# kcroker/Gadget-2.0.7-ngravs

Measured on AMD Instinct MI355X. Metric: particle-steps/s (tree+PM), higher is better.
Workload: dtype f64

## Files before the change

gadget-2.0.7-ngravs_amd/__init__.py:

```python
import ctypes as C
import os
import subprocess

import numpy as np

from . import abi, ic
from .abi import (Config, Particles, Stats, make_config, WALK_GROUP, WALK_STRICT,
                  LAW_NONE, LAW_NEWTON, LAW_NEG_NEWTON, LAW_YUKAWA, LAW_COLOYUK, LAW_BAMBAM, LAW_SOURCEBAM, LAW_TARGETBAM)

_HERE = os.path.dirname(os.path.abspath(__file__))
LIB_PATH = os.path.join(_HERE, "libngravs_hip.so")
_LIB = None

EXPORTS = [
    "ngravs_abi_version", "ngravs_build_info", "ngravs_config_default", "ngravs_create", "ngravs_create_with_laws", "ngravs_destroy",
    "ngravs_last_walk_kernel", "ngravs_last_pm_cus", "ngravs_cu_probe", "ngravs_shortrange_table_with_laws", "ngravs_user_table_eval",
    "ngravs_create_with_lattice", "ngravs_user_lattice_table",
    "ngravs_set_fatal_handler", "ngravs_set_opening", "ngravs_set_walk_mode", "ngravs_set_softening", "ngravs_dd_record_bytes", "ngravs_get_config", "ngravs_set_tuning",
    "ngravs_memcpy", "ngravs_device_alloc", "ngravs_device_free",
    "ngravs_set_particles",
    "ngravs_set_old_acc", "ngravs_update_particles", "ngravs_force_update_tree", "ngravs_domain_decomposition", "ngravs_discard_grav_pm",
    "ngravs_force_treebuild", "ngravs_gravity_tree",
    "ngravs_pmforce_periodic", "ngravs_compute_accelerations", "ngravs_get_accel", "ngravs_get_stats", "ngravs_walk_unopened",
    "ngravs_get_domain", "ngravs_get_keys", "ngravs_get_order", "ngravs_get_shard", "ngravs_last_error",
    "ngravs_peano_hilbert_key", "ngravs_peano_keys", "ngravs_shortrange_table", "ngravs_direct_sum", "ngravs_direct_sum_targets",
    "ngravs_dd_num_local", "ngravs_dd_local_extent", "ngravs_dd_set_extent", "ngravs_get_domain_extent", "ngravs_dd_set_toptree",
    "ngravs_dd_get_toptree", "ngravs_dd_peano_order", "ngravs_dd_leaf_sums", "ngravs_dd_target_bounds", "ngravs_dd_keep_margin", "ngravs_dd_pack", "ngravs_dd_get_dest",
    "ngravs_dd_pack_leaves", "ngravs_dd_set_top", "ngravs_dd_recv_buffer", "ngravs_dd_apply_migration", "ngravs_dd_set_halo",
    "ngravs_dd_leaf_sums_kept", "ngravs_dd_pack_leaves_kept", "ngravs_dd_refresh_halo", "ngravs_dd_update_top", "ngravs_dd_get_kept",
    "ngravs_dd_set_ids", "ngravs_dd_get_ids",
    "ngravs_pm_slab_begin", "ngravs_pm_slab_pack", "ngravs_pm_slab_unpack", "ngravs_pm_slab_bytes",
    "ngravs_sph_density", "ngravs_sph_kernel", "ngravs_sph_hydro",
]
HOST_EXPORTS = ["ngravs_host_comm_selftest", "ngravs_host_kept_step", "ngravs_host_toptree_borrow", "ngravs_host_domain_decomposition", "ngravs_host_domain_owners", "ngravs_host_domain_halo",
                "ngravs_host_plan_free", "ngravs_host_pmforce_periodic", "ngravs_host_compute_accelerations", "ngravs_host_split",
                "ngravs_host_pm_seconds", "ngravs_host_toptree_init", "ngravs_host_toptree_from_children", "ngravs_host_toptree_adapt",
                "ngravs_host_toptree_free", "ngravs_host_import_request", "ngravs_host_import_request_margin"]
RCCL_LIB_PATH = os.path.join(_HERE, "libngravs_rccl.so")
RCCL_EXPORTS = ["ngravs_rccl_selftest", "ngravs_rccl_unique_id", "ngravs_rccl_create", "ngravs_rccl_fill", "ngravs_rccl_destroy", "ngravs_rccl_stats",
                "ngravs_rccl_last_error", "ngravs_rccl_world", "ngravs_rccl_barrier", "ngravs_rccl_set_timeout"]


class NgravsError(RuntimeError):
    pass


def build(verbose=False):
    cmd = ["make", "-C", os.path.join(_HERE, "csrc"), "-j8"]
    if not verbose:
        cmd.insert(1, "-s")
    subprocess.check_call(cmd)
    return LIB_PATH


def lib():
    global _LIB
    if _LIB is None:
        if not os.path.exists(LIB_PATH):
            raise NgravsError("libngravs_hip.so is not built (run __graft_entry__.build()); there is no CPU fallback")
        L = C.CDLL(LIB_PATH)
        L.ngravs_build_info.restype = C.c_char_p
        L.ngravs_last_error.restype = C.c_char_p
        L.ngravs_last_error.argtypes = [C.c_void_p]
        L.ngravs_peano_hilbert_key.restype = C.c_int64
        L.ngravs_peano_hilbert_key.argtypes = [C.c_int] * 4
        L.ngravs_force_treebuild.restype = C.c_int64
        L.ngravs_force_treebuild.argtypes = [C.c_void_p]
        for name in ("ngravs_destroy", "ngravs_domain_decomposition", "ngravs_gravity_tree",
                     "ngravs_pmforce_periodic", "ngravs_discard_grav_pm"):
            getattr(L, name).argtypes = [C.c_void_p]
        L.ngravs_compute_accelerations.argtypes = [C.c_void_p, C.c_int]
        L.ngravs_set_opening.argtypes = [C.c_void_p, C.c_double, C.c_double]
        L.ngravs_set_walk_mode.argtypes = [C.c_void_p, C.c_int]
        L.ngravs_set_softening.argtypes = [C.c_void_p, C.c_void_p]
        L.ngravs_dd_record_bytes.restype = C.c_int64
        L.ngravs_dd_record_bytes.argtypes = [C.c_void_p, C.c_int]
        L.ngravs_set_particles.argtypes = [C.c_void_p, C.c_void_p]
        L.ngravs_set_old_acc.argtypes = [C.c_void_p, C.c_void_p, C.c_int64, C.c_int]
        L.ngravs_get_accel.argtypes = [C.c_void_p, C.c_void_p, C.c_int64, C.c_void_p, C.c_int64, C.c_void_p, C.c_int64,
                                       C.c_void_p, C.c_int64, C.c_int, C.c_int]
        L.ngravs_set_tuning.argtypes = [C.c_void_p, C.c_char_p, C.c_double]
        L.ngravs_memcpy.argtypes = [C.c_void_p, C.c_void_p, C.c_void_p, C.c_int64, C.c_int]
        L.ngravs_get_stats.argtypes = [C.c_void_p, C.c_void_p]
        L.ngravs_get_domain.argtypes = [C.c_void_p, C.c_void_p]
        L.ngravs_get_keys.argtypes = [C.c_void_p, C.c_void_p, C.c_int]
        L.ngravs_get_order.argtypes = [C.c_void_p, C.c_void_p, C.c_int]
        L.ngravs_get_shard.argtypes = [C.c_void_p, C.c_void_p, C.c_void_p]
        L.ngravs_peano_keys.argtypes = [C.c_void_p, C.c_void_p, C.c_int64, C.c_void_p, C.c_double, C.c_int, C.c_void_p]
        L.ngravs_shortrange_table.argtypes = [C.c_void_p, C.c_void_p, C.c_void_p]
        L.ngravs_direct_sum.argtypes = [C.c_void_p, C.c_void_p, C.c_int64, C.c_void_p]
        L.ngravs_direct_sum_targets.argtypes = [C.c_void_p, C.c_void_p, C.c_void_p, C.c_void_p, C.c_int64, C.c_void_p]
        L.ngravs_dd_local_extent.argtypes = [C.c_void_p, C.c_void_p, C.c_void_p]
        L.ngravs_dd_set_extent.argtypes = [C.c_void_p, C.c_void_p, C.c_void_p]
        L.ngravs_get_config.argtypes = [C.c_void_p, C.c_void_p]
        L.ngravs_host_split.argtypes = [C.c_void_p, C.c_void_p, C.c_int64, C.c_int, C.c_double, C.c_void_p]
        L.ngravs_dd_pack.argtypes = [C.c_void_p, C.c_int, C.c_void_p, C.c_int, C.c_int, C.c_void_p, C.c_void_p, C.c_void_p]
        L.ngravs_host_toptree_init.argtypes = [C.c_void_p, C.c_int]
        L.ngravs_host_toptree_from_children.argtypes = [C.c_void_p, C.c_void_p, C.c_int32]
        L.ngravs_host_toptree_adapt.argtypes = [C.c_void_p, C.c_void_p, C.c_double, C.c_int, C.c_void_p]
        L.ngravs_host_toptree_free.argtypes = [C.c_void_p]
        L.ngravs_host_toptree_free.restype = None
        L.ngravs_host_import_request.argtypes = [C.c_void_p, C.c_void_p, C.c_void_p, C.c_void_p, C.c_void_p, C.c_int, C.c_void_p, C.c_void_p]
        L.ngravs_dd_apply_migration.argtypes = [C.c_void_p, C.c_void_p, C.c_int64]
        L.ngravs_dd_set_halo.argtypes = [C.c_void_p, C.c_void_p, C.c_int64]
        L.ngravs_dd_set_ids.argtypes = [C.c_void_p, C.c_void_p, C.c_int]
        L.ngravs_create_with_laws.argtypes = [C.c_void_p, C.c_void_p, C.c_int, C.c_void_p]
        L.ngravs_last_walk_kernel.argtypes = [C.c_void_p]
        L.ngravs_last_pm_cus.argtypes = [C.c_void_p]
        L.ngravs_cu_probe.argtypes = [C.c_void_p, C.c_int, C.c_int, C.c_void_p]
        L.ngravs_shortrange_table_with_laws.argtypes = [C.c_void_p, C.c_void_p, C.c_int, C.c_void_p, C.c_void_p]
        L.ngravs_user_table_eval.argtypes = [C.c_void_p, C.c_double, C.c_double, C.c_double, C.c_void_p, C.c_int64, C.c_void_p,
                                             C.c_void_p]
        L.ngravs_dd_get_ids.argtypes = [C.c_void_p, C.c_void_p, C.c_int]
        L.ngravs_create_with_lattice.argtypes = [C.c_void_p, C.c_void_p, C.c_int, C.c_void_p, C.c_int, C.c_void_p]
        L.ngravs_user_lattice_table.argtypes = [abi.LATTICE_FN, C.c_double, C.c_void_p]
        L.ngravs_sph_density.argtypes = [C.c_void_p, C.c_void_p, C.c_void_p, C.c_void_p, C.c_void_p]
        L.ngravs_sph_kernel.argtypes = [C.c_double, C.c_void_p, C.c_int64, C.c_void_p, C.c_void_p]
        L.ngravs_sph_hydro.argtypes = [C.c_void_p, C.c_void_p, C.c_void_p, C.c_void_p]
        _LIB = L
    return _LIB


def shard_range(n, rank, world_size):
    lo = (n * rank) // world_size
    hi = (n * (rank + 1)) // world_size
    lo = (lo // 64) * 64
    hi = n if rank + 1 == world_size else (hi // 64) * 64
    return lo, hi - lo


def peano_hilbert_key(x, y, z, bits):
    return int(lib().ngravs_peano_hilbert_key(int(x), int(y), int(z), int(bits)))


def shortrange_table(cfg):
    ng = cfg.n_gravs
    force = np.zeros((ng, ng, abi.NTAB))
    pot = np.zeros((ng, ng, abi.NTAB))
    rc = lib().ngravs_shortrange_table(C.byref(cfg), force.ctypes.data, pot.ctypes.data)
    if rc != 0:
        raise NgravsError("ngravs_shortrange_table: %d" % rc)
    return force, pot


def shortrange_table_with_laws(cfg, user_fns):
    arr, nfns, keep = abi.user_registry(user_fns)
    ng = cfg.n_gravs
    force = np.zeros((ng, ng, abi.NTAB))
    pot = np.zeros((ng, ng, abi.NTAB))
    rc = lib().ngravs_shortrange_table_with_laws(C.byref(cfg), arr, nfns, force.ctypes.data, pot.ctypes.data)
    del keep
    if rc != 0:
        raise NgravsError("ngravs_shortrange_table_with_laws: %d" % rc)
    return force, pot


def user_table_eval(kind, fn, r, r_lo=0.0, r_hi=0.0, h=0.0):
    arr, _, keep = abi.user_registry([(kind, fn)])
    r = np.ascontiguousarray(r, dtype=np.float64)
    out = np.zeros_like(r)
    err = C.c_double(0)
    rc = lib().ngravs_user_table_eval(arr, r_lo, r_hi, h, r.ctypes.data, len(r), out.ctypes.data, C.byref(err))
    del keep
    if rc != 0:
        raise NgravsError("ngravs_user_table_eval: %d" % rc)
    return out, err.value


def user_lattice_table(fn, box_size):
    w = abi.lattice_fn(fn)
    out = np.zeros((3, abi.LAT_EN1, abi.LAT_EN1, abi.LAT_EN1))
    rc = lib().ngravs_user_lattice_table(w, float(box_size), out.ctypes.data)
    if rc != 0:
        msg = lib().ngravs_last_error(None)
        raise NgravsError("ngravs_user_lattice_table: %d: %s" % (rc, msg.decode() if msg else ""))
    return out


def sph_kernel(h, r):
    r = np.ascontiguousarray(r, dtype=np.float64)
    wk, dwk = np.zeros_like(r), np.zeros_like(r)
    rc = lib().ngravs_sph_kernel(float(h), r.ctypes.data, r.size, wk.ctypes.data, dwk.ctypes.data)
    if rc != 0:
        raise NgravsError("ngravs_sph_kernel: %d" % rc)
    return wk, dwk


def hydro_factors(time, omega0, omega_lambda, hubble, gamma=5.0 / 3):
    hubble_a = omega0 / (time * time * time) + (1 - omega0 - omega_lambda) / (time * time) + omega_lambda
    hubble_a = hubble * np.sqrt(hubble_a)
    hubble_a2 = time * time * hubble_a
    fac_mu = np.power(time, 3 * (gamma - 1) / 2) / time
    fac_vsic_fix = hubble_a * np.power(time, 3 * (gamma - 1))
    return float(hubble_a2), float(fac_mu), float(fac_vsic_fix)


def _ptr(a):
    return a.ctypes.data if a is not None else None


class Engine:

    def __init__(self, cfg, user_fns=None, user_lattice=None):
        self.cfg = cfg
        self._h = C.c_void_p()
        self._user_arr, nfns, self._user_keep = abi.user_registry(user_fns)
        self._lat_arr, nlat, self._lat_keep = abi.lattice_registry(user_lattice)
        rc = lib().ngravs_create_with_lattice(C.byref(cfg), self._user_arr, nfns, self._lat_arr, nlat, C.byref(self._h))
        if rc != 0:
            msg = lib().ngravs_last_error(None)
            self.status = rc
            raise NgravsError("ngravs_create failed with status %d (no HIP device or bad wiring): %s" % (rc, msg.decode() if msg else ""))
        self._keep = []
        self.n = 0

    def last_walk_kernel(self):
        return int(lib().ngravs_last_walk_kernel(self._h))

    def last_pm_cus(self):
        return int(lib().ngravs_last_pm_cus(self._h))

    def cu_probe(self, which, nblocks=2048):
        out = np.zeros(nblocks, dtype=np.int32)
        self._check(lib().ngravs_cu_probe(self._h, which, nblocks, out.ctypes.data), "ngravs_cu_probe")
        return out

    def close(self):
        if self._h:
            lib().ngravs_destroy(self._h)
            self._h = C.c_void_p()

    def __del__(self):
        try:
            self.close()
        except Exception:
            pass

    def _check(self, rc, what):
        if rc != 0:
            msg = lib().ngravs_last_error(self._h)
            raise NgravsError("%s failed: status %d (%s)" % (what, rc, msg.decode() if msg else ""))

    def _host_columns(self, pos, mass, ptype, old_acc, active, grav_pm, grav_cost=None):
        pos = np.ascontiguousarray(pos, dtype=np.float64)
        mass = np.ascontiguousarray(mass, dtype=np.float64)
        ptype = np.ascontiguousarray(ptype, dtype=np.int32)
        p = Particles()
        p.n = len(pos)
        p.pos, p.pos_stride = pos.ctypes.data, 24
        p.mass, p.mass_stride = mass.ctypes.data, 8
        p.type, p.type_stride = ptype.ctypes.data, 4
        keep = [pos, mass, ptype]
        if old_acc is not None:
            old_acc = np.ascontiguousarray(old_acc, dtype=np.float64)
            p.old_acc, p.old_acc_stride = old_acc.ctypes.data, 8
            keep.append(old_acc)
        if active is not None:
            active = np.ascontiguousarray(active, dtype=np.uint8)
            p.active, p.active_stride = active.ctypes.data, 1
            keep.append(active)
        if grav_pm is not None:
            grav_pm = np.ascontiguousarray(grav_pm, dtype=np.float64)
            p.grav_pm, p.grav_pm_stride = grav_pm.ctypes.data, 24
            keep.append(grav_pm)
        if grav_cost is not None:
            grav_cost = np.ascontiguousarray(grav_cost, dtype=np.float32)
            p.grav_cost, p.grav_cost_stride = grav_cost.ctypes.data, 4
            keep.append(grav_cost)
        p.on_device = 0
        self._keep = keep
        return p

    def set_particles(self, pos, mass, ptype, old_acc=None, active=None, grav_pm=None, grav_cost=None):
        p = self._host_columns(pos, mass, ptype, old_acc, active, grav_pm, grav_cost)
        self.n = p.n
        self._check(lib().ngravs_set_particles(self._h, C.byref(p)), "ngravs_set_particles")

    def update_particles(self, pos, mass, ptype, old_acc=None, active=None):
        p = self._host_columns(pos, mass, ptype, old_acc, active, None)
        self._check(lib().ngravs_update_particles(self._h, C.byref(p)), "ngravs_update_particles")

    def force_update_tree(self):
        self._check(lib().ngravs_force_update_tree(self._h), "ngravs_force_update_tree")

    def set_particles_device(self, n, pos_ptr, mass_ptr, type_ptr, old_acc_ptr=None, active_ptr=None, grav_pm_ptr=None):
        p = Particles()
        p.n = n
        p.pos, p.pos_stride = pos_ptr, 24
        p.mass, p.mass_stride = mass_ptr, 8
        p.type, p.type_stride = type_ptr, 4
        if old_acc_ptr:
            p.old_acc, p.old_acc_stride = old_acc_ptr, 8
        if active_ptr:
            p.active, p.active_stride = active_ptr, 1
        if grav_pm_ptr:
            p.grav_pm, p.grav_pm_stride = grav_pm_ptr, 24
        p.on_device = 1
        self.n = n
        self._check(lib().ngravs_set_particles(self._h, C.byref(p)), "ngravs_set_particles")

    def set_old_acc(self, old_acc):
        old_acc = np.ascontiguousarray(old_acc, dtype=np.float64)
        self._check(lib().ngravs_set_old_acc(self._h, old_acc.ctypes.data, 8, 0), "ngravs_set_old_acc")

    def set_old_acc_device(self, ptr):
        self._check(lib().ngravs_set_old_acc(self._h, ptr, 8, 1), "ngravs_set_old_acc")

    def get_old_acc_device(self, ptr):
        self._check(lib().ngravs_get_accel(self._h, None, 0, None, 0, ptr, 8, None, 0, 1, 0), "ngravs_get_accel")

    def get_accel_device(self, acc_ptr=None, pm_ptr=None, old_ptr=None, cost_ptr=None, only_active=False):
        self._check(lib().ngravs_get_accel(self._h, acc_ptr, 24, pm_ptr, 24, old_ptr, 8, cost_ptr, 4, 1, int(only_active)),
                    "ngravs_get_accel")

    def walk_unopened(self):
        v = C.c_int64(0)
        self._check(lib().ngravs_walk_unopened(self._h, C.byref(v)), "ngravs_walk_unopened")
        return int(v.value)

    def set_opening(self, theta, err_tol_force_acc):
        self._check(lib().ngravs_set_opening(self._h, theta, err_tol_force_acc), "ngravs_set_opening")
        self.cfg.err_tol_theta = theta
        self.cfg.err_tol_force_acc = err_tol_force_acc

    def set_softening(self, force_softening):
        fs = np.ascontiguousarray(force_softening, dtype=np.float64)
        assert fs.shape == (6,)
        self._check(lib().ngravs_set_softening(self._h, fs.ctypes.data), "ngravs_set_softening")
        for t in range(6):
            self.cfg.force_softening[t] = fs[t]

    def set_walk_mode(self, mode):
        self._check(lib().ngravs_set_walk_mode(self._h, mode), "ngravs_set_walk_mode")

    def set_tuning(self, **kw):
        for k, v in kw.items():
            self._check(lib().ngravs_set_tuning(self._h, k.encode(), float(v)), "ngravs_set_tuning(%s)" % k)

    def domain_Decomposition(self):
        self._check(lib().ngravs_domain_decomposition(self._h), "domain_Decomposition")

    def force_treebuild(self):
        nn = lib().ngravs_force_treebuild(self._h)
        if nn < 0:
            self._check(int(nn), "force_treebuild")
        return int(nn)

    def gravity_tree(self):
        self._check(lib().ngravs_gravity_tree(self._h), "gravity_tree")

    def pmforce_periodic(self):
        self._check(lib().ngravs_pmforce_periodic(self._h), "pmforce_periodic")

    def compute_accelerations(self, pm_step=True):
        self._check(lib().ngravs_compute_accelerations(self._h, 1 if pm_step else 0), "compute_accelerations")

    def get_accel(self, want_pm=False, into=None):
        n = self.n
        if into is not None:
            acc, old, cost = into
            assert acc.dtype == np.float64 and old.dtype == np.float64 and cost.dtype == np.float32
            assert acc.flags.c_contiguous and old.flags.c_contiguous and cost.flags.c_contiguous
        else:
            acc = np.zeros((n, 3))
            old = np.zeros(n)
            cost = np.zeros(n, dtype=np.float32)
        pm = np.zeros((n, 3)) if want_pm else None
        self._check(lib().ngravs_get_accel(self._h, acc.ctypes.data, 24, _ptr(pm), 24, old.ctypes.data, 8,
                                           cost.ctypes.data, 4, 0, 1 if into is not None else 0), "ngravs_get_accel")
        return (acc, old, cost, pm) if want_pm else (acc, old, cost)

    def get_pm(self):
        pm = np.zeros((self.n, 3))
# ... 131 lines not shown
```

gadget-2.0.7-ngravs_amd/csrc/capi.hip:

```cpp
#include "engine.hpp"
#include "../../include/ngravs_peano.h"
#include <chrono>
#include <cmath>

static thread_local std::string g_create_error;

void ngravs_report(ngravs_ctx *ctx, int code, const std::string &msg)
{
  if(ctx)
    ctx->last_error = msg;
  else
    g_create_error = msg;
  if(ctx && ctx->on_fatal)
    ctx->on_fatal(code, msg.c_str());
  else
    fprintf(stderr, "task %d: endrun called with an error level of %d (%s)\n", ctx ? ctx->cfg.rank : 0, code, msg.c_str());
}

__global__ void k_pack_strided_f64(const unsigned char *src, long long stride, int ncomp, long long n, double *dst)
{
  long long i = blockIdx.x * (long long)blockDim.x + threadIdx.x;
  if(i >= n)
    return;
  const double *s = reinterpret_cast<const double *>(src + i * stride);
// ... 235 lines not shown
extern "C" int ngravs_create_with_laws(const ngravs_config_t *cfg, const ngravs_user_fn_t *fns, int nfns, ngravs_ctx **out)
{
  return ngravs_create_with_lattice(cfg, fns, nfns, nullptr, 0, out);
}

extern "C" int ngravs_create_with_lattice(const ngravs_config_t *cfg, const ngravs_user_fn_t *fns, int nfns,
                                          const ngravs_user_lattice_t *lat, int nlat, ngravs_ctx **out)
{
  if(!cfg || !out)
    return NGRAVS_ERR_ARG;
  *out = nullptr;
  std::string why;
  int rc = check_config(cfg, why);
  if(rc == NGRAVS_OK)
    rc = user_check_config(cfg, fns, nfns, lat, nlat, why);
  if(rc != NGRAVS_OK)
    {
      ngravs_report(nullptr, rc, why);
      return rc;
    }
  int ndev = 0;
  if(hipGetDeviceCount(&ndev) != hipSuccess || ndev <= 0)
    {
      ngravs_report(nullptr, NGRAVS_ERR_NO_DEVICE, "no HIP device: libngravs_hip has no CPU fallback");
      return NGRAVS_ERR_NO_DEVICE;
    }
  if(cfg->device < 0 || cfg->device >= ndev)
    return NGRAVS_ERR_ARG;
  ngravs_ctx *c = new ngravs_ctx;
  c->cfg = *cfg;
  c->user_fns.assign(fns, fns + nfns);
  c->user_lat.assign(lat, lat + nlat);
  memset(&c->stats, 0, sizeof(c->stats));
  if(hipSetDevice(cfg->device) != hipSuccess || hipStreamCreate(&c->stream) != hipSuccess ||
     hipEventCreate(&c->ev0) != hipSuccess || hipEventCreate(&c->ev1) != hipSuccess ||
     hipEventCreate(&c->evk0) != hipSuccess || hipEventCreate(&c->evk1) != hipSuccess || hipEventCreate(&c->ev_fork) != hipSuccess ||
     hipEventCreate(&c->ev_pm0) != hipSuccess || hipEventCreate(&c->ev_pm1) != hipSuccess || hipEventCreate(&c->ev_walk) != hipSuccess)
    {
      delete c;
      return NGRAVS_ERR_NO_DEVICE;
    }
  if(cfg->pmgrid)
    {
      c->asmth = cfg_asmth(cfg);
      c->rcut = cfg_rcut(cfg);
    }
  *out = c;
  return NGRAVS_OK;
}

extern "C" void ngravs_destroy(ngravs_ctx *c)
{
  if(!c)
    return;
  (void)hipSetDevice(c->cfg.device);
  (void)hipStreamSynchronize(c->stream);
  pm_release(c);
  pmslab_release(c);
  c->in_cost.release();
  c->in_pos.release();
  c->in_mass.release();
  c->in_oldacc.release();
  c->in_type.release();
  c->in_active.release();
  c->in_key.release();
  c->in_rec.release();
  c->in_id.release();
  c->dd_mask.release();
  c->dd_counts.release();
  c->dd_send.release();
  c->dd_recv.release();
  c->top.child.release();
  c->top.leaf.release();
  c->top.gcnt.release();
  c->top.info.release();
  c->top.gsum.release();
  c->top.leaf_owner.release();
  c->top.reqmask.release();
  c->top.leaf_sums.release();
  ngravs_host_toptree_free(&c->top.h);
  c->n_top.release();
  c->s_pm.release();
  c->s_type.release();
  c->s_active.release();
  c->s_oldacc.release();
  c->s_key.release();
  c->s_idx.release();
  c->idx_iota.release();
  c->sort_tmp.release();
  c->red_tmp.release();
  c->n_first.release();
  c->n_count.release();
  c->n_child.release();
  c->n_flags.release();
  c->n_nchild.release();
  c->n_geo.release();
  c->n_mom.release();
  c->n_npart.release();
  c->user_tab.release();
  c->user_green.release();
  c->scan_out.release();
  c->tb_count.release();
  c->scan_tmp.release();
  c->d_counters.release();
  c->d_levels.release();
  c->table.release();
  c->lat.release();
  c->walk_stack.release();
  c->walk_counters.release();
  c->walk_ovf.release();
  c->walk_tlist.release();
  c->walk_tmp.release();
  c->lvl_table.release();
  c->r_acc.release();
  c->r_pm.release();
  c->r_oldacc.release();
  c->r_nint.release();
  c->pm_rho.release();
  c->pm_phi.release();
  c->pm_force.release();
  c->pm_orig.release();
  c->out_tmp.release();
  c->out_tmpf.release();
  c->sph_vel_in.release();
  c->sph_h_in.release();
  c->sph_vel.release();
  c->sph_tlist.release();
  c->sph_tmp.release();
  c->sph_res.release();
  c->sph_row.release();
  c->sph_rounds.release();
  c->sph_counters.release();
  c->sph_col_in.release();
  c->sph_ts_in.release();
  c->sph_hsrc.release();
  c->sph_hmax.release();
  (void)hipEventDestroy(c->ev0);
  (void)hipEventDestroy(c->ev1);
  (void)hipEventDestroy(c->evk0);
  (void)hipEventDestroy(c->evk1);
  for(hipEvent_t e : c->ev_batch)
    (void)hipEventDestroy(e);
  (void)hipEventDestroy(c->ev_fork);
  (void)hipEventDestroy(c->ev_pm0);
  (void)hipEventDestroy(c->ev_pm1);
  (void)hipEventDestroy(c->ev_walk);
  if(c->pm_stream)
    {
      (void)hipStreamSynchronize(c->pm_stream);
      (void)hipStreamSynchronize(c->walk_stream);
      (void)hipStreamDestroy(c->pm_stream);
      (void)hipStreamDestroy(c->walk_stream);
    }
  c->probe_out.release();
  (void)hipStreamDestroy(c->stream);
  delete c;
}

extern "C" void ngravs_set_fatal_handler(ngravs_ctx *ctx, ngravs_fatal_fn fn)
{
  if(ctx)
    ctx->on_fatal = fn;
}

extern "C" int ngravs_set_opening(ngravs_ctx *c, double theta, double errtol)
{
  if(!c)
    return NGRAVS_ERR_ARG;
  c->cfg.err_tol_theta = theta;
  c->cfg.err_tol_force_acc = errtol;
  return NGRAVS_OK;
}

extern "C" int ngravs_set_softening(ngravs_ctx *c, const double force_softening[NGRAVS_NTYPES])
{
  if(!c || !force_softening)
    return NGRAVS_ERR_ARG;
  for(int t = 0; t < NGRAVS_NTYPES; t++)
    if(!(force_softening[t] >= 0.0))
      {
        ngravs_report(c, NGRAVS_ERR_ARG, "ngravs_set_softening: negative or NaN softening length");
        return NGRAVS_ERR_ARG;
      }
  for(int t = 0; t < NGRAVS_NTYPES; t++)
    c->cfg.force_softening[t] = force_softening[t];
  return NGRAVS_OK;
}

extern "C" int ngravs_set_walk_mode(ngravs_ctx *c, int mode)
{
  if(!c || (mode != NGRAVS_WALK_STRICT && mode != NGRAVS_WALK_GROUP))
    return NGRAVS_ERR_ARG;
  c->cfg.walk_mode = mode;
  return NGRAVS_OK;
}

extern "C" int ngravs_get_config(ngravs_ctx *c, ngravs_config_t *out)
{
  if(!c || !out)
    return NGRAVS_ERR_ARG;
  *out = c->cfg;
  if(c->cfg.pmgrid)
    {
      out->asmth = c->asmth;
      out->rcut = c->rcut;
    }
  return NGRAVS_OK;
}

extern "C" int ngravs_set_tuning(ngravs_ctx *c, const char *name, double v)
{
  if(!c || !name)
    return NGRAVS_ERR_ARG;
  const std::string k(name);
  const long long iv = (long long)v;
  Tuning &t = c->tune;
  if(k == "walk_fused")
    t.walk_fused = iv != 0;
  else if(k == "walk_batch" && iv >= 0)
    t.walk_batch = iv;
  else if(k == "walk_waves" && iv >= 0 && iv <= 16)
    t.walk_waves = (int)iv;
  else if(k == "walk_lcap" && (iv == 0 || (iv >= 1024 && iv <= 65536)))
    {
      t.walk_lcap = (int)iv;
      c->walk_lcap = 0;
    }
  else if(k == "walk_root")
    t.walk_root = iv != 0;
  else if(k == "walk_compact")
    t.walk_compact = iv != 0;
  else if(k == "walk_spread" && iv >= 0 && iv <= 64 && (iv & (iv - 1)) == 0)
    t.walk_spread = (int)iv;
  else if(k == "walk_sg" && iv >= 0 && iv <= 16)
    t.walk_sg = (int)iv;
  else if(k == "walk_ring" && iv >= 0 && iv <= 1)
    t.walk_ring = (int)iv;
  else if(k == "walk_ring_k" && iv >= 0 && iv <= 8)
    t.walk_ring_k = (int)iv;
  else if(k == "walk_nleaf" && iv >= -1 && iv <= 8)
    t.walk_nleaf = (int)iv;
  else if(k == "walk_exact_reach")
    t.walk_exact_reach = iv != 0;
  else if(k == "sort_full")
    t.sort_full = iv != 0;
  else if(k == "tree_levelwise")
    t.tree_levelwise = iv != 0;
  else if(k == "dd_keep" && v >= 0 && v <= 0.25)
    t.dd_keep = v;
  else if(k == "pm_cus" && (iv == -1 || (iv >= 0 && iv <= 32 && iv % 8 == 0)))
    t.pm_cus = (int)iv;
  else if(k == "sph_verbose")
    t.sph_verbose = iv != 0;
  else
    {
      ngravs_report(c, NGRAVS_ERR_ARG, "ngravs_set_tuning: unknown name or value out of range: " + k);
      return NGRAVS_ERR_ARG;
    }
  return NGRAVS_OK;
}

extern "C" int ngravs_memcpy(ngravs_ctx *c, void *dst, const void *src, int64_t bytes, int kind)
{
  if(!c || bytes < 0 || kind < 1 || kind > 3 || (bytes > 0 && (!dst || !src)))
    return NGRAVS_ERR_ARG;
  if(bytes == 0)
    return NGRAVS_OK;
  (void)hipSetDevice(c->cfg.device);
  HIP_TRY(c, hipStreamSynchronize(c->stream));
  HIP_TRY(c, hipMemcpy(dst, src, (size_t)bytes, kind == 1 ? hipMemcpyHostToDevice : (kind == 2 ? hipMemcpyDeviceToHost : hipMemcpyDeviceToDevice)));
  return NGRAVS_OK;
}

extern "C" int ngravs_device_alloc(ngravs_ctx *c, void **ptr, int64_t bytes)
{
  if(!c || !ptr || bytes < 0)
    return NGRAVS_ERR_ARG;
  *ptr = nullptr;
  (void)hipSetDevice(c->cfg.device);
  if(hipMalloc(ptr, (size_t)(bytes > 0 ? bytes : 1)) != hipSuccess)
    return NGRAVS_ERR_NOMEM;
  return NGRAVS_OK;
}

extern "C" int ngravs_device_free(ngravs_ctx *c, void *ptr)
{
  if(!c)
    return NGRAVS_ERR_ARG;
  (void)hipSetDevice(c->cfg.device);
  if(ptr)
    (void)hipFree(ptr);
  return NGRAVS_OK;
}

static int upload_column_f64(ngravs_ctx *c, const void *src, int64_t stride, int ncomp, int64_t n, int on_device, double *dst)
{
  if(on_device)
    {
      if(stride == (int64_t)sizeof(double) * ncomp)
        HIP_TRY(c, hipMemcpyAsync(dst, src, sizeof(double) * ncomp * n, hipMemcpyDeviceToDevice, c->stream));
      else
        hipLaunchKernelGGL(k_pack_strided_f64, GRID1(n), 0, c->stream, (const unsigned char *)src, (long long)stride, ncomp,
                           (long long)n, dst);
      return NGRAVS_OK;
    }
  if(stride == (int64_t)sizeof(double) * ncomp)
    {
      HIP_TRY(c, hipMemcpyAsync(dst, src, sizeof(double) * ncomp * n, hipMemcpyHostToDevice, c->stream));
      HIP_TRY(c, hipStreamSynchronize(c->stream));
      return NGRAVS_OK;
    }
  c->host_stage.resize(sizeof(double) * ncomp * (size_t)n);
  double *h = reinterpret_cast<double *>(c->host_stage.data());
  for(int64_t i = 0; i < n; i++)
    memcpy(h + i * ncomp, (const unsigned char *)src + i * stride, sizeof(double) * ncomp);
  HIP_TRY(c, hipMemcpyAsync(dst, h, sizeof(double) * ncomp * n, hipMemcpyHostToDevice, c->stream));
  HIP_TRY(c, hipStreamSynchronize(c->stream));
  return NGRAVS_OK;
}

static double ev_ms(ngravs_ctx *c);

static int set_particles_impl(ngravs_ctx *c, const ngravs_particles_t *p, bool keep_tree)
{
  if(!c || !p || p->n < 0 || (p->n > 0 && (!p->pos || !p->mass || !p->type)))
    return NGRAVS_ERR_ARG;
  if(p->n == 0 && keep_tree)
    {
      if(!c->have_particles || c->n_local != 0)
        return NGRAVS_ERR_STATE;
      c->tree_stale = c->have_tree;
      return NGRAVS_OK;
    }
  if(p->n == 0)
    {
      (void)hipSetDevice(c->cfg.device);
      c->n = c->n_local = 0;
      c->own_order_nlocal = -1;
      c->sort_low = 35;
      c->all_active = true;
      c->walk_ia_ratio = 0;
      c->pm_solo_steps = 0, c->pm_auto_cus = -1;
      c->walk_unit_state = 4;
      c->have_particles = true;
      c->have_order = c->have_tree = c->have_pm = c->have_acc = false;
      c->top.on = false;
      c->pm_parked = false;
      return NGRAVS_OK;
    }
  const bool keep_halo = keep_tree && c->n_local != c->n;
  if(keep_tree && (!c->have_order || !c->have_tree || p->n != c->n_local))
    {
      ngravs_report(c, NGRAVS_ERR_STATE, "ngravs_update_particles: needs a built tree over the same own particles");
      return NGRAVS_ERR_STATE;
    }
  if(p->n >= (1ll << 31) - 64)
    {
      ngravs_report(c, NGRAVS_ERR_ARG, "int particle indices (reference All.MaxPart is int): n must be < 2^31");
      return NGRAVS_ERR_ARG;
    }
  (void)hipSetDevice(c->cfg.device);
  const int64_t n = p->n;
  if(c->in_pos.ensure(3 * n) || c->in_mass.ensure(n) || c->in_oldacc.ensure(n) || c->in_type.ensure(n) || c->in_active.ensure(n) ||
     (!keep_tree && c->in_cost.ensure(n)))
    {
      ngravs_report(c, NGRAVS_ERR_NOMEM, "device allocation failed");
      return NGRAVS_ERR_NOMEM;
    }
  if(!keep_halo)
    c->n = n;
  c->n_local = n;
  if(!keep_tree)
    {
      if(c->own_order_nlocal != n)
        c->own_order_nlocal = -1;
      c->sort_low = 35;
    }
  int rc;
  if(!keep_tree && (rc = dd_fill_ids(c)))
    return rc;
  if((rc = upload_column_f64(c, p->pos, p->pos_stride, 3, n, p->on_device, c->in_pos.p)))
    return rc;
  if((rc = upload_column_f64(c, p->mass, p->mass_stride, 1, n, p->on_device, c->in_mass.p)))
    return rc;
  if(p->old_acc)
    {
      if((rc = upload_column_f64(c, p->old_acc, p->old_acc_stride, 1, n, p->on_device, c->in_oldacc.p)))
        return rc;
    }
  else
    hipLaunchKernelGGL(k_fill_f64, GRID1(n), 0, c->stream, c->in_oldacc.p, (long long)n, 0.0);
  if(!keep_tree)
    {
      if(p->grav_cost && p->on_device)
        hipLaunchKernelGGL(k_pack_strided_f32_to_f64, GRID1(n), 0, c->stream, (const unsigned char *)p->grav_cost,
                           (long long)p->grav_cost_stride, (long long)n, c->in_cost.p);
      else if(p->grav_cost)
        {
          c->host_stage.resize(sizeof(double) * (size_t)n);
          double *h = reinterpret_cast<double *>(c->host_stage.data());
          for(int64_t i = 0; i < n; i++)
            {
              float f;
              memcpy(&f, (const unsigned char *)p->grav_cost + i * p->grav_cost_stride, sizeof(float));
              h[i] = f;
            }
          HIP_TRY(c, hipMemcpyAsync(c->in_cost.p, h, sizeof(double) * n, hipMemcpyHostToDevice, c->stream));
          HIP_TRY(c, hipStreamSynchronize(c->stream));
        }
      else
        hipLaunchKernelGGL(k_fill_f64, GRID1(n), 0, c->stream, c->in_cost.p, (long long)n, 0.0);
    }
  if(p->on_device)
    {
      if(c->d_counters.ensure(16))
        return NGRAVS_ERR_NOMEM;
      int nbad = 0;
      HIP_TRY(c, hipMemsetAsync(c->d_counters.p + 15, 0, sizeof(int), c->stream));
      hipLaunchKernelGGL(k_pack_type, GRID1(n), 0, c->stream, (const unsigned char *)p->type, (long long)p->type_stride,
                         (long long)n, c->in_type.p, c->d_counters.p + 15);
      HIP_TRY(c, hipMemcpyAsync(&nbad, c->d_counters.p + 15, sizeof(int), hipMemcpyDeviceToHost, c->stream));
      HIP_TRY(c, hipStreamSynchronize(c->stream));
      if(nbad)
        {
          ngravs_report(c, NGRAVS_ERR_ARG, "particle Type outside 0..5");
          return NGRAVS_ERR_ARG;
        }
    }
  else
    {
      c->host_stage.resize(sizeof(int) * (size_t)n);
      int *h = reinterpret_cast<int *>(c->host_stage.data());
      for(int64_t i = 0; i < n; i++)
        {
          memcpy(h + i, (const unsigned char *)p->type + i * p->type_stride, sizeof(int));
          if(h[i] < 0 || h[i] >= NGRAVS_NTYPES)
            {
              ngravs_report(c, NGRAVS_ERR_ARG, "particle Type outside 0..5");
              return NGRAVS_ERR_ARG;
            }
        }
      HIP_TRY(c, hipMemcpyAsync(c->in_type.p, h, sizeof(int) * n, hipMemcpyHostToDevice, c->stream));
      HIP_TRY(c, hipStreamSynchronize(c->stream));
    }
  c->all_active = p->active == nullptr;
  if(p->active)
    {
      if(p->on_device)
        hipLaunchKernelGGL(k_pack_active, GRID1(n), 0, c->stream, (const unsigned char *)p->active,
                           (long long)p->active_stride, (long long)n, c->in_active.p);
      else
        {
          c->host_stage.resize((size_t)n);
          for(int64_t i = 0; i < n; i++)
            c->host_stage[i] = ((const unsigned char *)p->active)[i * p->active_stride] ? 1 : 0;
          HIP_TRY(c, hipMemcpyAsync(c->in_active.p, c->host_stage.data(), (size_t)n, hipMemcpyHostToDevice, c->stream));
          HIP_TRY(c, hipStreamSynchronize(c->stream));
        }
    }
  else
    hipLaunchKernelGGL(k_fill_u8, GRID1(n), 0, c->stream, c->in_active.p, (long long)n, (unsigned char)1);
  HIP_TRY(c, hipGetLastError());
  c->walk_ia_ratio = 0;
  c->pm_solo_steps = 0, c->pm_auto_cus = -1;
  c->walk_unit_state = 4;
  c->have_particles = true;
  if(keep_tree)
    c->tree_stale = true;
  else
    {
      c->have_order = c->have_tree = c->have_pm = c->have_acc = false;
      c->top.on = false;
      c->pm_parked = false;
      if(p->grav_pm && c->cfg.pmgrid)
        {
          if(c->pm_orig.ensure(3 * n))
            return NGRAVS_ERR_NOMEM;
          if((rc = upload_column_f64(c, p->grav_pm, p->grav_pm_stride, 3, n, p->on_device, c->pm_orig.p)))
            return rc;
          c->pm_parked = true;
        }
    }
  return NGRAVS_OK;
}

extern "C" int ngravs_set_particles(ngravs_ctx *c, const ngravs_particles_t *p) { return set_particles_impl(c, p, false); }

extern "C" int ngravs_update_particles(ngravs_ctx *c, const ngravs_particles_t *p) { return set_particles_impl(c, p, true); }

extern "C" int ngravs_force_update_tree(ngravs_ctx *c)
{
  if(!c || !c->have_order || !c->have_tree)
    return NGRAVS_ERR_STATE;
  (void)hipSetDevice(c->cfg.device);
  if(c->n == 0)
    {
      c->tree_stale = false;
      return NGRAVS_OK;
    }
  HIP_TRY(c, hipEventRecord(c->ev0, c->stream));
  int rc = dom_regather(c);
  if(rc)
    return rc;
  if((rc = tree_moments(c, true)))
    return rc;
  HIP_TRY(c, hipEventRecord(c->ev1, c->stream));
  c->stats.t_treebuild = ev_ms(c) * 1e-3;
  c->stats.t_domain = c->stats.t_peano = 0;
  c->tree_stale = false;
  c->tree_refit = true;
  return NGRAVS_OK;
}

extern "C" int ngravs_set_old_acc(ngravs_ctx *c, const double *old_acc, int64_t stride, int on_device)
{
  if(!c || !c->have_particles || !old_acc)
    return NGRAVS_ERR_ARG;
  (void)hipSetDevice(c->cfg.device);
  if(c->n_local == 0)
    return NGRAVS_OK;
  int rc = upload_column_f64(c, old_acc, stride, 1, c->n_local, on_device, c->in_oldacc.p);
  if(rc)
    return rc;
  if(c->have_order)
    hipLaunchKernelGGL(k_permute_f64, GRID1(c->n), 0, c->stream, c->s_idx.p, (long long)c->n, 1, c->in_oldacc.p, c->s_oldacc.p);
  HIP_TRY(c, hipGetLastError());
  return NGRAVS_OK;
}

static double ev_ms(ngravs_ctx *c)
{
  float ms = 0;
  (void)hipEventSynchronize(c->ev1);
  (void)hipEventElapsedTime(&ms, c->ev0, c->ev1);
  return ms;
}

static int park_grav_pm(ngravs_ctx *c)
{
  if(!c->have_pm || !c->have_order)
    return NGRAVS_OK;
  if(c->pm_orig.ensure(3 * (c->n_local > 0 ? c->n_local : 1)))
    return NGRAVS_ERR_NOMEM;
  hipLaunchKernelGGL(k_unpermute_f64_lim, GRID1(c->n), 0, c->stream, c->s_idx.p, (long long)c->n, (long long)c->n_local, 3, c->r_pm.p,
                     c->pm_orig.p);
  c->pm_parked = true;
  c->have_pm = false;
  return NGRAVS_OK;
}

static int domain_decomposition_impl(ngravs_ctx *c, bool keep_pm)
{
  if(!c || !c->have_particles)
    return NGRAVS_ERR_STATE;
  (void)hipSetDevice(c->cfg.device);
  if(keep_pm)
    {
      if(int rc = park_grav_pm(c))
        return rc;
    }
  else
    c->pm_parked = false;
  c->have_pm = c->pm_parked;
  c->pm_parked = false;
  if(c->n == 0)
    {
      c->own_order_nlocal = -1;
      c->shard_first = c->shard_count = 0;
      c->have_order = true;
      c->have_tree = c->tree_stale = c->have_pm = false;
      c->stats.t_domain = c->stats.t_peano = 0;
      return NGRAVS_OK;
    }
  HIP_TRY(c, hipEventRecord(c->ev0, c->stream));
  int rc = dom_find_extent(c);
  if(rc)
    return rc;
  HIP_TRY(c, hipEventRecord(c->ev1, c->stream));
  c->stats.t_domain = ev_ms(c) * 1e-3;
  HIP_TRY(c, hipEventRecord(c->ev0, c->stream));
  c->own_order_nlocal = -1;
  rc = dom_keys_and_sort(c);
  if(rc)
    return rc;
  c->own_order_nlocal = c->n_local;
  c->own_order_len = c->n;
  HIP_TRY(c, hipEventRecord(c->ev1, c->stream));
  c->stats.t_peano = ev_ms(c) * 1e-3;
  int64_t ws = c->cfg.world_size, r = c->cfg.rank;
  int64_t lo = (c->n * r) / ws, hi = (c->n * (r + 1)) / ws;
  lo = (lo / 64) * 64;
  hi = (r + 1 == ws) ? c->n : (hi / 64) * 64;
  c->shard_first = lo;
  c->shard_count = hi - lo;
  c->have_order = true;
  c->have_tree = false;
  c->tree_stale = false;
  if(c->have_pm)
    {
      if(c->r_pm.ensure(3 * c->n))
        return NGRAVS_ERR_NOMEM;
      hipLaunchKernelGGL(k_permute_f64_lim, GRID1(c->n), 0, c->stream, c->s_idx.p, (long long)c->n, (long long)c->n_local, 3, c->pm_orig.p,
                         c->r_pm.p);
      HIP_TRY(c, hipGetLastError());
    }
  return NGRAVS_OK;
}

extern "C" int ngravs_domain_decomposition(ngravs_ctx *c) { return domain_decomposition_impl(c, true); }

extern "C" int ngravs_discard_grav_pm(ngravs_ctx *c)
{
  if(!c)
    return NGRAVS_ERR_ARG;
  c->have_pm = false;
  c->pm_parked = false;
  return NGRAVS_OK;
}

extern "C" int64_t ngravs_force_treebuild(ngravs_ctx *c)
{
  if(!c || !c->have_order)
    return NGRAVS_ERR_STATE;
  (void)hipSetDevice(c->cfg.device);
  if(c->n == 0)
    {
      c->nnodes = 0;
      c->have_tree = true;
      c->tree_refit = false;
      c->stats.t_treebuild = 0;
      return 0;
    }
  if(hipEventRecord(c->ev0, c->stream) != hipSuccess)
    return NGRAVS_ERR_NO_DEVICE;
  int rc = tree_build(c);
  if(rc)
    return rc;
  if(hipEventRecord(c->ev1, c->stream) != hipSuccess)
    return NGRAVS_ERR_NO_DEVICE;
  c->stats.t_treebuild = ev_ms(c) * 1e-3;
  c->have_tree = true;
  c->tree_refit = false;
  return c->nnodes;
}

static int ensure_table(ngravs_ctx *c)
{
  if(!c->cfg.pmgrid || c->table_ready)
    return NGRAVS_OK;
  const int ng = c->cfg.n_gravs;
  std::vector<double> h((size_t)(ng * ng + 1) * NTAB);
  host_shortrange_table(&c->cfg, h.data(), nullptr, c->user_fns.data(), (int)c->user_fns.size());
  {
    WalkParams wp;
    make_walk_params(c, &wp);
    for(int t = 0; t < NTAB; t++)
      h[(size_t)ng * ng * NTAB + t] = exp(-wp.ym * (double)t * wp.inv_asmthfac);
  }
  if(c->table.ensure(h.size()))
    return NGRAVS_ERR_NOMEM;
  HIP_TRY(c, hipMemcpyAsync(c->table.p, h.data(), sizeof(double) * h.size(), hipMemcpyHostToDevice, c->stream));
  HIP_TRY(c, hipStreamSynchronize(c->stream));
  c->table_ready = true;
  return NGRAVS_OK;
}

static bool pm_cu_bit(int R, int b)
{
  const int x = b / 32, k = b - 33 * x;
  return b < 256 && k >= 0 && k % 8 == 0 && k / 8 < R / 8;
}

static int masked_streams(ngravs_ctx *c, int R)
{
  if(c->pm_stream && c->pm_stream_cus == R)
    return NGRAVS_OK;
  if(!c->device_cus)
    {
      hipDeviceProp_t prop;
      HIP_TRY(c, hipGetDeviceProperties(&prop, c->cfg.device));
      c->device_cus = prop.multiProcessorCount;
    }
  if(c->device_cus != 256 || R < 8 || R > 32 || R % 8)
    return NGRAVS_ERR_ARG;
  if(c->pm_stream)
    {
      HIP_TRY(c, hipStreamSynchronize(c->pm_stream));
      HIP_TRY(c, hipStreamSynchronize(c->walk_stream));
      (void)hipStreamDestroy(c->pm_stream);
      (void)hipStreamDestroy(c->walk_stream);
      c->pm_stream = c->walk_stream = nullptr;
      c->pm_stream_cus = 0;
    }
  uint32_t mp[8] = {0}, mw[8] = {0};
  for(int b = 0; b < 256; b++)
    (pm_cu_bit(R, b) ? mp : mw)[b / 32] |= 1u << (b % 32);
  hipStream_t sp = nullptr, sw = nullptr;
  if(hipExtStreamCreateWithCUMask(&sp, 8, mp) != hipSuccess || hipExtStreamCreateWithCUMask(&sw, 8, mw) != hipSuccess)
    {
      if(sp)
        (void)hipStreamDestroy(sp);
      (void)hipGetLastError();
      return NGRAVS_ERR_NO_DEVICE;
    }
  uint32_t gp[8] = {0}, gw[8] = {0};
  if(hipExtStreamGetCUMask(sp, 8, gp) != hipSuccess || hipExtStreamGetCUMask(sw, 8, gw) != hipSuccess || memcmp(gp, mp, sizeof mp) ||
     memcmp(gw, mw, sizeof mw))
    {
      (void)hipStreamDestroy(sp);
      (void)hipStreamDestroy(sw);
      (void)hipGetLastError();
      return NGRAVS_ERR_NO_DEVICE;
    }
  c->pm_stream = sp;
  c->walk_stream = sw;
  c->pm_stream_cus = R;
  return NGRAVS_OK;
}

static bool overlap_eligible(const ngravs_ctx *c)
{
  return c->cfg.pmgrid && c->cfg.periodic && c->cfg.world_size == 1 && !c->top.on && c->cfg.walk_mode == NGRAVS_WALK_GROUP &&
         c->n > 0 && c->n_local > 0;
}

static int gravity_tree_impl(ngravs_ctx *c, hipEvent_t pm_done)
{
  if(!c || !c->have_order)
    return NGRAVS_ERR_STATE;
  (void)hipSetDevice(c->cfg.device);
  int rc;
  if(!c->have_tree)
    {
      int64_t nn = ngravs_force_treebuild(c);
      if(nn < 0)
        return (int)nn;
    }
  else if(c->tree_stale && (rc = ngravs_force_update_tree(c)))
    return rc;
  if((rc = ensure_table(c)))
    return rc;
  if(c->n_local == 0)
    {
      c->stats.t_treewalk = 0;
      c->stats.walk_kernel_ms = 0;
      c->stats.interactions = 0;
      c->stats.n_active = 0;
      c->have_acc = true;
      return NGRAVS_OK;
    }
  HIP_TRY(c, hipEventRecord(c->ev0, c->stream));
  const bool masked = (pm_done || (c->tune.pm_cus > 0 && overlap_eligible(c))) && masked_streams(c, pm_done ? c->pm_stream_cus : c->tune.pm_cus) == NGRAVS_OK;
  if(masked)
    {
      HIP_TRY(c, hipStreamWaitEvent(c->walk_stream, c->ev0, 0));
      {
        OnStream on(c, c->walk_stream, c->device_cus - c->pm_stream_cus);
        if((rc = walk_run(c)))
          return rc;
      }
      HIP_TRY(c, hipEventRecord(c->ev_walk, c->walk_stream));
      HIP_TRY(c, hipStreamWaitEvent(c->stream, c->ev_walk, 0));
    }
  else if((rc = walk_run(c)))
    return rc;
  if(pm_done)
    HIP_TRY(c, hipStreamWaitEvent(c->stream, pm_done, 0));
  if((rc = walk_finish(c)))
    return rc;
  HIP_TRY(c, hipEventRecord(c->ev1, c->stream));
  c->stats.t_treewalk = ev_ms(c) * 1e-3;
  float kms = 0;
  (void)hipEventSynchronize(c->evk1);
  (void)hipEventElapsedTime(&kms, c->evk0, c->evk1);
  c->stats.walk_kernel_ms = kms;
  double h[2] = {0, 0};
  HIP_TRY(c, hipMemcpyAsync(h, c->red_tmp.p, 2 * sizeof(double), hipMemcpyDeviceToHost, c->stream));
  HIP_TRY(c, hipStreamSynchronize(c->stream));
  c->stats.interactions = h[0];
  c->stats.n_active = (int64_t)h[1];
  c->have_acc = true;
  if(c->cfg.pmgrid && c->cfg.walk_mode == NGRAVS_WALK_GROUP && h[1] > 0 && c->cfg.box_size > 0)
    {
      const double reach = (c->cfg.group_reach > 0 ? c->cfg.group_reach : NGRAVS_GROUP_REACH) * c->asmth;
      const double ntot = c->top.on && c->top.total_count > 0 ? c->top.total_count : (double)c->n;
      const double L = c->cfg.box_size, expect = 4.18879020478639 * reach * reach * reach * ntot / (L * L * L);
      const bool dense = c->walk_ntargets < 0 || c->walk_dense_tlist;
      if(expect > 0 && dense)
        {
          const double f_sg = c->walk_sg >= 4 ? 1.0 : (c->walk_sg >= 2 ? 1857.0 / 1393.0 : 1857.0 / 1079.0);
          const double f_s = c->walk_spread >= 2 ? 1079.0 / 871.0 : 1.0;
          c->walk_ia_ratio = (h[0] / h[1]) / expect * f_sg * f_s;
        }
    }
  if(c->shard_count > 0 && c->extent_override)
    hipLaunchKernelGGL(k_cost_update, GRID1(c->shard_count), 0, c->stream, c->s_idx.p, c->s_active.p, c->r_nint.p,
                       (long long)c->shard_first, (long long)c->shard_count, c->in_cost.p);
  return NGRAVS_OK;
}

extern "C" int ngravs_gravity_tree(ngravs_ctx *c) { return gravity_tree_impl(c, nullptr); }

static int pm_on_masked_stream(ngravs_ctx *c)
{
  HIP_TRY(c, hipEventRecord(c->ev_fork, c->stream));
  HIP_TRY(c, hipStreamWaitEvent(c->pm_stream, c->ev_fork, 0));
  OnStream on(c, c->pm_stream, c->pm_stream_cus);
  HIP_TRY(c, hipEventRecord(c->ev_pm0, c->stream));
  int rc = pm_run(c);
  if(rc)
    return rc;
  HIP_TRY(c, hipEventRecord(c->ev_pm1, c->stream));
  return NGRAVS_OK;
}

extern "C" int ngravs_pmforce_periodic(ngravs_ctx *c)
{
  if(!c || !c->have_particles)
    return NGRAVS_ERR_STATE;
  (void)hipSetDevice(c->cfg.device);
  int rc;
  if(!c->have_order && (rc = ngravs_domain_decomposition(c)))
    return rc;
  if(!c->have_tree)
    {
      int64_t nn = ngravs_force_treebuild(c);
      if(nn < 0)
        return (int)nn;
    }
  else if(c->tree_stale && (rc = ngravs_force_update_tree(c)))
    return rc;
  if(c->tune.pm_cus > 0 && overlap_eligible(c) && masked_streams(c, c->tune.pm_cus) == NGRAVS_OK)
    {
      if((rc = pm_on_masked_stream(c)))
        return rc;
      float ms = 0;
      HIP_TRY(c, hipEventSynchronize(c->ev_pm1));
      (void)hipEventElapsedTime(&ms, c->ev_pm0, c->ev_pm1);
      HIP_TRY(c, hipStreamWaitEvent(c->stream, c->ev_pm1, 0));
      c->stats.t_pm = ms * 1e-3;
      return NGRAVS_OK;
    }
  HIP_TRY(c, hipEventRecord(c->ev0, c->stream));
  if((rc = pm_run(c)))
    return rc;
  HIP_TRY(c, hipEventRecord(c->ev1, c->stream));
  c->stats.t_pm = ev_ms(c) * 1e-3;
  return NGRAVS_OK;
}

static const double PM_CU_SCALE[4] = {17.75, 9.07, 6.16, 4.74};
static const double PM_FIT_MARGIN = 1.05, PM_SHARE_COST = 1.04;
static int choose_pm_cus(ngravs_ctx *c)
{
  if(!overlap_eligible(c))
    return 0;
  if(c->tune.pm_cus >= 0)
    return c->tune.pm_cus;
  if(c->pm_auto_cus >= 0)
    return c->pm_auto_cus;
  if(c->pm_solo_steps < 2 || c->pm_solo_ms <= 0 || c->walk_solo_ms <= 0)
    return 0;
  c->pm_auto_cus = 0;
  for(int m = 1; m <= 4; m++)
    {
      const double walk = c->walk_solo_ms * 256.0 / (256 - 8 * m);
      if(c->pm_solo_ms * PM_CU_SCALE[m - 1] * PM_FIT_MARGIN < walk)
        {
          if(walk * PM_SHARE_COST < 0.99 * (c->pm_solo_ms + c->walk_solo_ms))
            c->pm_auto_cus = 8 * m;
          break;
        }
    }
  return c->pm_auto_cus;
}

extern "C" int ngravs_compute_accelerations(ngravs_ctx *c, int pm_step)
{
  if(!c || !c->have_particles)
    return NGRAVS_ERR_STATE;
  int rc;
  if((rc = domain_decomposition_impl(c, !(pm_step && c->cfg.pmgrid))))
    return rc;
  c->last_pm_cus = 0;
  if(!(pm_step && c->cfg.pmgrid))
    return ngravs_gravity_tree(c);
  const int R = choose_pm_cus(c);
  if(R > 0 && masked_streams(c, R) == NGRAVS_OK)
    {
      int64_t nn = ngravs_force_treebuild(c);
      if(nn < 0)
        return (int)nn;
      if((rc = pm_on_masked_stream(c)))
        return rc;
      if((rc = gravity_tree_impl(c, c->ev_pm1)))
        return rc;
      float ms = 0;
      (void)hipEventElapsedTime(&ms, c->ev_pm0, c->ev_pm1);
      c->stats.t_pm = ms * 1e-3;
      c->last_pm_cus = R;
      if(c->tune.pm_cus < 0 && ms > c->stats.walk_kernel_ms)
        c->pm_auto_cus = R < 32 ? R + 8 : 0;
      return NGRAVS_OK;
    }
  if((rc = ngravs_pmforce_periodic(c)))
    return rc;
  if((rc = ngravs_gravity_tree(c)))
    return rc;
  if(overlap_eligible(c) && c->tune.pm_cus < 0 && c->pm_auto_cus < 0)
    {
      c->pm_solo_ms = c->stats.t_pm * 1e3;
      c->walk_solo_ms = c->stats.walk_kernel_ms;
      c->pm_solo_steps++;
    }
  return NGRAVS_OK;
}

static int download_strided(ngravs_ctx *c, const void *dsrc, size_t elem, int ncomp, int64_t n, void *dst, int64_t stride,
                            int on_device)
{
  const size_t row = elem * ncomp;
  if(on_device)
    {
      if((size_t)stride != row)
        {
          ngravs_report(c, NGRAVS_ERR_ARG, "device outputs must be contiguous");
          return NGRAVS_ERR_ARG;
        }
      HIP_TRY(c, hipMemcpyAsync(dst, dsrc, row * n, hipMemcpyDeviceToDevice, c->stream));
      HIP_TRY(c, hipStreamSynchronize(c->stream));
      return NGRAVS_OK;
    }
  if((size_t)stride == row)
    {
      HIP_TRY(c, hipMemcpyAsync(dst, dsrc, row * n, hipMemcpyDeviceToHost, c->stream));
      HIP_TRY(c, hipStreamSynchronize(c->stream));
      return NGRAVS_OK;
    }
  c->host_stage.resize(row * (size_t)n);
  HIP_TRY(c, hipMemcpyAsync(c->host_stage.data(), dsrc, row * n, hipMemcpyDeviceToHost, c->stream));
  HIP_TRY(c, hipStreamSynchronize(c->stream));
  for(int64_t i = 0; i < n; i++)
    memcpy((unsigned char *)dst + i * stride, c->host_stage.data() + i * row, row);
  return NGRAVS_OK;
}

static int deliver(ngravs_ctx *c, const void *dsrc, size_t elem, int ncomp, int64_t n, void *dst, int64_t stride, int on_device,
                   const unsigned char *d_mask)
{
  if(!d_mask)
    return download_strided(c, dsrc, elem, ncomp, n, dst, stride, on_device);
  const size_t row = elem * ncomp;
  if(on_device)
    {
      if((size_t)stride != row)
        {
          ngravs_report(c, NGRAVS_ERR_ARG, "device outputs must be contiguous");
          return NGRAVS_ERR_ARG;
        }
      if(elem == sizeof(double))
        hipLaunchKernelGGL(k_copy_masked_f64, GRID1(n), 0, c->stream, d_mask, (long long)n, ncomp, (const double *)dsrc, (double *)dst);
      else
        hipLaunchKernelGGL(k_copy_masked_f32, GRID1(n), 0, c->stream, d_mask, (long long)n, (const float *)dsrc, (float *)dst);
      HIP_TRY(c, hipStreamSynchronize(c->stream));
      return NGRAVS_OK;
    }
  c->host_stage.resize(row * (size_t)n + (size_t)n);
  unsigned char *hm = c->host_stage.data() + row * (size_t)n;
  HIP_TRY(c, hipMemcpyAsync(c->host_stage.data(), dsrc, row * n, hipMemcpyDeviceToHost, c->stream));
  HIP_TRY(c, hipMemcpyAsync(hm, d_mask, (size_t)n, hipMemcpyDeviceToHost, c->stream));
  HIP_TRY(c, hipStreamSynchronize(c->stream));
  for(int64_t i = 0; i < n; i++)
    if(hm[i] & 1)
      memcpy((unsigned char *)dst + i * stride, c->host_stage.data() + i * row, row);
  return NGRAVS_OK;
}

extern "C" int ngravs_get_accel(ngravs_ctx *c, double *grav_accel, int64_t accel_stride, double *grav_pm, int64_t pm_stride,
                                double *old_acc, int64_t old_acc_stride, float *grav_cost, int64_t cost_stride, int on_device,
                                int only_active)
{
  if(!c || !c->have_order)
    return NGRAVS_ERR_STATE;
  (void)hipSetDevice(c->cfg.device);
  const int64_t n = c->n, nl = c->n_local;
  if(nl == 0)
    return NGRAVS_OK;
  if(c->out_tmp.ensure(3 * n) || c->out_tmpf.ensure(n))
    return NGRAVS_ERR_NOMEM;
  const unsigned char *mask = only_active ? c->in_active.p : nullptr;
  int rc;
  if(grav_accel)
    {
      if(!c->have_acc)
        return NGRAVS_ERR_STATE;
      HIP_TRY(c, hipMemsetAsync(c->out_tmp.p, 0, sizeof(double) * 3 * n, c->stream));
      hipLaunchKernelGGL(k_unpermute_f64, GRID1(n), 0, c->stream, c->s_idx.p, (long long)n, 3, c->r_acc.p, c->out_tmp.p);
      if((rc = deliver(c, c->out_tmp.p, sizeof(double), 3, nl, grav_accel, accel_stride, on_device, mask)))
        return rc;
    }
  if(grav_pm)
    {
      if(!c->have_pm)
        return NGRAVS_ERR_STATE;
      hipLaunchKernelGGL(k_unpermute_f64, GRID1(n), 0, c->stream, c->s_idx.p, (long long)n, 3, c->r_pm.p, c->out_tmp.p);
      if((rc = deliver(c, c->out_tmp.p, sizeof(double), 3, nl, grav_pm, pm_stride, on_device, nullptr)))
        return rc;
    }
  if(old_acc)
    {
      if(!c->have_acc)
        return NGRAVS_ERR_STATE;
      hipLaunchKernelGGL(k_unpermute_f64, GRID1(n), 0, c->stream, c->s_idx.p, (long long)n, 1, c->r_oldacc.p, c->out_tmp.p);
      if((rc = deliver(c, c->out_tmp.p, sizeof(double), 1, nl, old_acc, old_acc_stride, on_device, mask)))
        return rc;
    }
  if(grav_cost)
    {
      if(!c->have_acc)
        return NGRAVS_ERR_STATE;
      hipLaunchKernelGGL(k_unpermute_i2f, GRID1(n), 0, c->stream, c->s_idx.p, (long long)n, c->r_nint.p, c->out_tmpf.p);
      if((rc = deliver(c, c->out_tmpf.p, sizeof(float), 1, nl, grav_cost, cost_stride, on_device, mask)))
        return rc;
    }
  return NGRAVS_OK;
}

extern "C" int ngravs_get_stats(ngravs_ctx *c, ngravs_stats_t *out)
{
  if(!c || !out)
    return NGRAVS_ERR_ARG;
  *out = c->stats;
  return NGRAVS_OK;
}

static std::string kept_state(const ngravs_ctx *c, const char *who)
{
  char b[320];
  snprintf(b, sizeof(b), "%s: no kept decomposition to work on (own rows %lld, rows at the cut %lld, working set %lld, tree %d, top %d, task %d of %d)", who,
           (long long)c->n_local, (long long)c->top.own_leaf_n, (long long)c->n, (int)c->have_tree, (int)c->top.on, c->top.kept_rank, c->top.kept_world);
  return std::string(b);
}
extern "C" int ngravs_dd_leaf_sums_kept(ngravs_ctx *c, void **dev_sums, int64_t *count)
{
  if(!c || !dev_sums || !count)
    return NGRAVS_ERR_ARG;
  (void)hipSetDevice(c->cfg.device);
  const int rc = dd_leaf_sums_kept(c, dev_sums, count);
  if(rc == NGRAVS_ERR_STATE)
    ngravs_report(c, rc, kept_state(c, "ngravs_dd_leaf_sums_kept"));
  return rc;
}
extern "C" int ngravs_dd_pack_leaves_kept(ngravs_ctx *c, int64_t *counts, void **dev_records, int64_t *nrec)
{
  if(!c || !counts || !dev_records || !nrec)
    return NGRAVS_ERR_ARG;
  (void)hipSetDevice(c->cfg.device);
  const int rc = dd_pack_leaves_kept(c, counts, dev_records, nrec);
  if(rc == NGRAVS_ERR_STATE)
    ngravs_report(c, rc, kept_state(c, "ngravs_dd_pack_leaves_kept"));
  return rc;
}
extern "C" int ngravs_dd_refresh_halo(ngravs_ctx *c, const void *dev_records, int64_t nrec)
{
  if(!c || nrec < 0 || (nrec > 0 && !dev_records))
    return NGRAVS_ERR_ARG;
  (void)hipSetDevice(c->cfg.device);
  const int rc = dd_refresh_halo(c, dev_records, nrec);
  if(rc == NGRAVS_ERR_STATE)
    ngravs_report(c, rc, kept_state(c, "ngravs_dd_refresh_halo"));
  return rc;
}
extern "C" int ngravs_dd_update_top(ngravs_ctx *c, const double *node_sums, const double *leaf_len)
{
  if(!c)
    return NGRAVS_ERR_ARG;
  (void)hipSetDevice(c->cfg.device);
  const int rc = dd_update_top(c, node_sums, leaf_len);
  if(rc == NGRAVS_ERR_STATE)
    ngravs_report(c, rc, kept_state(c, "ngravs_dd_update_top"));
  return rc;
}
extern "C" int ngravs_dd_get_kept(ngravs_ctx *c, int32_t *rank, int32_t *world, const int32_t **leaf_owner, const uint8_t **present,
                                  const double **node_sums)
{
  if(!c)
    return NGRAVS_ERR_ARG;
  const TopTree &t = c->top;
  if(!(t.on && t.h.nnode > 0 && t.own_leaf_n == c->n_local && t.kept_rank >= 0 && (int)t.h_leaf_owner.size() == t.h.nleaf &&
       (int)t.h_present.size() == t.h.nleaf))
    {
      ngravs_report(c, NGRAVS_ERR_STATE, kept_state(c, "ngravs_dd_get_kept"));
      return NGRAVS_ERR_STATE;
    }
  if(rank)
    *rank = t.kept_rank;
  if(world)
    *world = t.kept_world;
  if(leaf_owner)
    *leaf_owner = t.h_leaf_owner.data();
  if(present)
    *present = t.h_present.data();
  if(node_sums)
    *node_sums = t.h_node_sums.data();
  return NGRAVS_OK;
}

extern "C" int ngravs_walk_unopened(ngravs_ctx *c, int64_t *count)
{
  if(!c || !count)
    return NGRAVS_ERR_ARG;
  *count = (int64_t)c->walk_unopened;
  return NGRAVS_OK;
}

extern "C" int ngravs_get_domain(ngravs_ctx *c, double out[8])
{
  if(!c || !c->have_order)
    return NGRAVS_ERR_STATE;
  memcpy(out, c->dom, sizeof(double) * 8);
  return NGRAVS_OK;
}

extern "C" int ngravs_get_keys(ngravs_ctx *c, int64_t *keys, int on_device)
{
  if(!c || !c->have_order || !keys)
    return NGRAVS_ERR_STATE;
  (void)hipSetDevice(c->cfg.device);
  const int64_t n = c->n;
  if(c->out_tmp.ensure(3 * n))
    return NGRAVS_ERR_NOMEM;
  long long *tmp = reinterpret_cast<long long *>(c->out_tmp.p);
  hipLaunchKernelGGL(k_key18, GRID1(n), 0, c->stream, c->in_key.p, (long long)n, tmp);
  return download_strided(c, tmp, sizeof(long long), 1, c->n_local, keys, sizeof(long long), on_device);
}

extern "C" int ngravs_get_order(ngravs_ctx *c, int32_t *order, int on_device)
{
  if(!c || !c->have_order || !order)
    return NGRAVS_ERR_STATE;
  (void)hipSetDevice(c->cfg.device);
  return download_strided(c, c->s_idx.p, sizeof(int), 1, c->n, order, sizeof(int), on_device);
}

extern "C" int ngravs_get_shard(ngravs_ctx *c, int64_t *first, int64_t *count)
{
  if(!c || !c->have_order)
    return NGRAVS_ERR_STATE;
  if(first)
    *first = c->shard_first;
  if(count)
    *count = c->shard_count;
  return NGRAVS_OK;
}

extern "C" const char *ngravs_last_error(ngravs_ctx *c) { return c ? c->last_error.c_str() : g_create_error.c_str(); }
extern "C" int ngravs_last_walk_kernel(ngravs_ctx *c) { return c ? c->last_walk_kernel : NGRAVS_ERR_ARG; }
extern "C" int ngravs_last_pm_cus(ngravs_ctx *c) { return c ? c->last_pm_cus : NGRAVS_ERR_ARG; }

#define CU_PROBE_LDS (96 * 1024)
__global__ void k_cu_probe(int *out, int n)
{
  extern __shared__ int probe_lds[];
  if(threadIdx.x != 0)
    return;
  unsigned xcc = 0, hw = 0;
  asm volatile("s_getreg_b32 %0, hwreg(HW_REG_XCC_ID)" : "=s"(xcc));
  asm volatile("s_getreg_b32 %0, hwreg(HW_REG_HW_ID)" : "=s"(hw));
  probe_lds[0] = (int)(((xcc & 15u) << 8) | ((hw >> 8) & 0xffu));
  const unsigned long long t0 = wall_clock64();
  while(wall_clock64() - t0 < 2000)
    __builtin_amdgcn_s_sleep(8);
  if((int)blockIdx.x < n)
    out[blockIdx.x] = probe_lds[0];
}

extern "C" int ngravs_cu_probe(ngravs_ctx *c, int which, int nblocks, int32_t *cu_ids)
{
  if(!c || !cu_ids || nblocks < 1 || nblocks > 65536 || which < 0 || which > 2)
    return NGRAVS_ERR_ARG;
  if(which > 0 && !c->pm_stream)
    return NGRAVS_ERR_STATE;
  (void)hipSetDevice(c->cfg.device);
  hipStream_t s = which == 0 ? c->stream : (which == 1 ? c->pm_stream : c->walk_stream);
  if(c->probe_out.ensure((size_t)nblocks))
    return NGRAVS_ERR_NOMEM;
  HIP_TRY(c, hipFuncSetAttribute(reinterpret_cast<const void *>(k_cu_probe), hipFuncAttributeMaxDynamicSharedMemorySize, CU_PROBE_LDS));
  hipLaunchKernelGGL(k_cu_probe, dim3((unsigned)nblocks), dim3(64), CU_PROBE_LDS, s, c->probe_out.p, nblocks);
  HIP_TRY(c, hipGetLastError());
  HIP_TRY(c, hipMemcpyAsync(cu_ids, c->probe_out.p, sizeof(int) * nblocks, hipMemcpyDeviceToHost, s));
  HIP_TRY(c, hipStreamSynchronize(s));
  return NGRAVS_OK;
}

extern "C" int64_t ngravs_peano_hilbert_key(int x, int y, int z, int bits) { return ngravs_ph_key(x, y, z, bits); }

extern "C" int ngravs_peano_keys(ngravs_ctx *c, const double *pos, int64_t n, const double corner[3], double fac, int bits,
                                 int64_t *keys)
{
  if(!c || !pos || !keys || n <= 0 || bits < 1 || bits > 21)
    return NGRAVS_ERR_ARG;
  (void)hipSetDevice(c->cfg.device);
  DevBuf<double> dpos;
  DevBuf<long long> dkeys;
  if(dpos.ensure(3 * n) || dkeys.ensure(n))
    return NGRAVS_ERR_NOMEM;
  int rc = NGRAVS_OK;
  if(hipMemcpyAsync(dpos.p, pos, sizeof(double) * 3 * n, hipMemcpyHostToDevice, c->stream) != hipSuccess)
    rc = NGRAVS_ERR_NO_DEVICE;
  if(!rc)
    rc = dom_keys_only(c, dpos.p, n, corner, fac, bits, dkeys.p);
  if(!rc && hipMemcpyAsync(keys, dkeys.p, sizeof(long long) * n, hipMemcpyDeviceToHost, c->stream) != hipSuccess)
    rc = NGRAVS_ERR_NO_DEVICE;
  (void)hipStreamSynchronize(c->stream);
  dpos.release();
  dkeys.release();
  return rc;
}

extern "C" int ngravs_shortrange_table(const ngravs_config_t *cfg, double *force_out, double *pot_out)
{
  if(!cfg || !force_out || cfg->n_gravs < 1 || cfg->n_gravs > NGRAVS_MAX_GRAVS)
    return NGRAVS_ERR_ARG;
  host_shortrange_table(cfg, force_out, pot_out);
  return NGRAVS_OK;
}

extern "C" int ngravs_shortrange_table_with_laws(const ngravs_config_t *cfg, const ngravs_user_fn_t *fns, int nfns, double *force_out,
                                                 double *pot_out)
{
  if(!cfg || !force_out || cfg->n_gravs < 1 || cfg->n_gravs > NGRAVS_MAX_GRAVS || nfns < 0 || nfns > NGRAVS_MAX_USER_FNS ||
     (nfns > 0 && !fns))
    return NGRAVS_ERR_ARG;
  for(int i = 0; i < cfg->n_gravs; i++)
    for(int j = 0; j < cfg->n_gravs; j++)
      {
        const int law = cfg->law_normed[i][j], k = law - NGRAVS_LAW_USER0;
        if(law >= NGRAVS_LAW_USER0 && (k >= nfns || fns[k].kind != NGRAVS_USER_NORMED || !fns[k].fn))
          return NGRAVS_ERR_WIRING;
      }
  host_shortrange_table(cfg, force_out, pot_out, fns, nfns);
  return NGRAVS_OK;
}

extern "C" int ngravs_direct_sum(ngravs_ctx *c, const int32_t *idx, int64_t nt, double *acc)
{
  if(!c || !c->have_order || !idx || !acc || nt <= 0)
    return NGRAVS_ERR_STATE;
  (void)hipSetDevice(c->cfg.device);
  DevBuf<int> inv, din, dout;
  DevBuf<double> dacc;
  if(inv.ensure(c->n) || din.ensure(nt) || dout.ensure(nt) || dacc.ensure(3 * nt))
    return NGRAVS_ERR_NOMEM;
  int rc = NGRAVS_OK;
  hipLaunchKernelGGL(k_inverse_perm, GRID1(c->n), 0, c->stream, c->s_idx.p, (long long)c->n, inv.p);
  if(hipMemcpyAsync(din.p, idx, sizeof(int) * nt, hipMemcpyHostToDevice, c->stream) != hipSuccess)
    rc = NGRAVS_ERR_NO_DEVICE;
  hipLaunchKernelGGL(k_map_idx, GRID1(nt), 0, c->stream, inv.p, din.p, (long long)nt, dout.p);
  if(!rc)
    rc = direct_run(c, dout.p, nt, dacc.p);
  if(!rc && hipMemcpyAsync(acc, dacc.p, sizeof(double) * 3 * nt, hipMemcpyDeviceToHost, c->stream) != hipSuccess)
    rc = NGRAVS_ERR_NO_DEVICE;
  (void)hipStreamSynchronize(c->stream);
  inv.release();
  din.release();
  dout.release();
  dacc.release();
  return rc;
}

extern "C" int ngravs_direct_sum_targets(ngravs_ctx *c, const double *pos, const double *mass, const int32_t *type, int64_t nt, double *acc)
{
  if(!c || !c->have_order || !pos || !type || !acc || nt <= 0)
    return NGRAVS_ERR_STATE;
  for(int64_t k = 0; k < nt; k++)
    if(type[k] < 0 || type[k] >= NGRAVS_NTYPES)
      return NGRAVS_ERR_ARG;
  (void)hipSetDevice(c->cfg.device);
  DevBuf<double4> dt;
  DevBuf<int> dty;
  DevBuf<double> dacc;
  if(dt.ensure(nt) || dty.ensure(nt) || dacc.ensure(3 * nt))
    return NGRAVS_ERR_NOMEM;
  std::vector<double4> h((size_t)nt);
  double r_need = 0;
  for(int64_t k = 0; k < nt; k++)
    {
      h[k].x = pos[3 * k];
      h[k].y = pos[3 * k + 1];
      h[k].z = pos[3 * k + 2];
      h[k].w = mass ? mass[k] : 1.0;
      const double dx = h[k].x - c->dom[3], dy = h[k].y - c->dom[4], dz = h[k].z - c->dom[5];
      r_need = fmax(r_need, 1.25 * (sqrt(dx * dx + dy * dy + dz * dz) + 0.5 * sqrt(3.0) * c->dom[6]));
    }
  int rc = NGRAVS_OK;
  if(hipMemcpyAsync(dt.p, h.data(), sizeof(double4) * nt, hipMemcpyHostToDevice, c->stream) != hipSuccess ||
     hipMemcpyAsync(dty.p, type, sizeof(int) * nt, hipMemcpyHostToDevice, c->stream) != hipSuccess)
    rc = NGRAVS_ERR_NO_DEVICE;
  if(!rc)
    rc = direct_run_targets(c, dt.p, dty.p, nt, dacc.p, r_need);
  if(!rc && hipMemcpyAsync(acc, dacc.p, sizeof(double) * 3 * nt, hipMemcpyDeviceToHost, c->stream) != hipSuccess)
    rc = NGRAVS_ERR_NO_DEVICE;
  (void)hipStreamSynchronize(c->stream);
  dt.release();
  dty.release();
  dacc.release();
  return rc;
}

extern "C" int64_t ngravs_dd_num_local(ngravs_ctx *c) { return c ? c->n_local : NGRAVS_ERR_ARG; }

// ... 455 lines not shown
```

gadget-2.0.7-ngravs_amd/csrc/engine.hpp:

```cpp
#pragma once
#include <hip/hip_runtime.h>
#include <cstdint>
#include <cstdio>
#include <cstdlib>
#include <cstring>
#include <string>
#include <vector>
#include "../../include/ngravs_host.h"

#define NG_MAX NGRAVS_MAX_GRAVS
#define NTAB NGRAVS_NTAB
#define TREE_BITS NGRAVS_TREE_BITS
#define FLAG_BUCKET 64
#define FLAG_PSEUDO 128
#define FLAG_PARTIAL 256
#define MAX_LEVELS (TREE_BITS + 1)

struct ngravs_ctx;

#define HIP_TRY(ctx, expr)                                                                        \
  do                                                                                              \
    {                                                                                             \
      hipError_t e__ = (expr);                                                                    \
      if(e__ != hipSuccess)                                                                       \
        {                                                                                         \
          ngravs_report(ctx, NGRAVS_ERR_NO_DEVICE, std::string(#expr) + ": " + hipGetErrorString(e__)); \
          return NGRAVS_ERR_NO_DEVICE;                                                            \
        }                                                                                         \
    }                                                                                             \
  while(0)

void ngravs_report(ngravs_ctx *ctx, int code, const std::string &msg);

template <typename T> struct DevBuf
{
  T *p = nullptr;
  size_t cap = 0;
  int ensure(size_t n)
  {
    if(n <= cap)
      return 0;
    if(p)
      (void)hipFree(p);
    p = nullptr;
    cap = 0;
    size_t want = n + n / 16 + 64;
    if(hipMalloc((void **)&p, want * sizeof(T)) != hipSuccess)
      return -1;
    cap = want;
    return 0;
  }
  void release()
  {
    if(p)
      (void)hipFree(p);
    p = nullptr;
    cap = 0;
  }
};

#define UL_NC 8
struct UserTabs
{
  const double *coef, *spl;
  int e_lo, n_oct, S;
  int nh, Ss;
  double h[NGRAVS_NTYPES];
};
__host__ __device__ inline double ul_poly(const double *c, double t)
{
  double v = c[7];
  for(int j = 6; j >= 0; j--)
    v = v * t + c[j];
  return v;
}
__host__ __device__ inline double ul_g(const UserTabs &u, int k, double r)
{
  int e;
  (void)frexp(r, &e);
  int o = e - u.e_lo;
  const double m = ldexp(r, -(u.e_lo + (o < 0 ? 0 : (o >= u.n_oct ? u.n_oct - 1 : o))));
  double s = (m - 0.5) * (2 * u.S);
  s = o < 0 ? 0.0 : (o >= u.n_oct ? (double)u.S : s);
  o = o < 0 ? 0 : (o >= u.n_oct ? u.n_oct - 1 : o);
  s = s >= 0 ? (s <= u.S ? s : (double)u.S) : 0.0;
  int j = (int)s;
  j = j >= u.S ? u.S - 1 : j;
  return ul_poly(u.coef + ((size_t)(k * u.n_oct + o) * u.S + j) * UL_NC, 2 * (s - j) - 1);
}
__host__ __device__ inline double ul_spline(const UserTabs &u, int k, double h, double r)
{
  if(u.nh == 0)
    return 0.0;
  int i = 0;
  for(int q = 1; q < u.nh; q++)
    if(fabs(u.h[q] - h) < fabs(u.h[i] - h))
      i = q;
  double s = r / h * u.Ss;
  s = s >= 0 ? (s <= u.Ss ? s : (double)u.Ss) : 0.0;
  int j = (int)s;
  j = j >= u.Ss ? u.Ss - 1 : j;
  return ul_poly(u.spl + ((size_t)(k * u.nh + i) * u.Ss + j) * UL_NC, 2 * (s - j) - 1);
}

struct WalkParams
{
  int ng, periodic, pm, use_theta;
  int nleaf;
  int exact_reach;
  double box, boxhalf;
  double theta2;
  double errtol_acc;
  double rcut, rcut2, asmthfac, utor2wpi, reach2;
  double ym;
  double bam_eps;
  double fac_intp;
  double fsoft[NGRAVS_NTYPES];
  int t2g[NGRAVS_NTYPES];
  unsigned t2g_packed;
  double cN[NG_MAX][NG_MAX], cY[NG_MAX][NG_MAX], cS[NG_MAX][NG_MAX];
  int ntab_lds;
  int tab_slot[NG_MAX * NG_MAX];
  int slot_src[NG_MAX * NG_MAX];
  int exp_tab;
  double inv_asmthfac;
  double ec[4];
  int src_in_box;
  int bam;
  int law_accel[NG_MAX][NG_MAX], law_spline[NG_MAX][NG_MAX];
  int user;
  UserTabs ut;
};

struct TreeView
{
  const int *first, *count, *child, *flags;
  const int *npart;
  const double4 *geo, *mom;
  int nnodes;
  const int *ltab;
  int ltab_level;
  double ltab_corner[3], ltab_cl;
};

struct Tuning
{
  int walk_fused = 0, walk_waves = 0, walk_lcap = 0, walk_root = 0, walk_compact = 1, walk_spread = 0, walk_exact_reach = 0, walk_sg = 0, walk_nleaf = -1;
  long long walk_batch = 0;
  int sort_full = 0;
  int tree_levelwise = 0;
  double dd_keep = 0;
  int walk_ring = 1;
  int walk_ring_k = 0;
  int pm_cus = -1;
  int sph_verbose = 0;
};

#define TOP_CW(ng) (7 + 4 * (ng))
struct TopTree
{
  double total_count = 0;
  bool on = false;
  double import_reach = 0;
  ngravs_toptree h = {0, 0, 0, 0, nullptr, nullptr, nullptr, nullptr, nullptr};
  DevBuf<int> child, leaf;
  DevBuf<int> gcnt;
  DevBuf<unsigned char> info;
  DevBuf<double> gsum;
  DevBuf<int> leaf_owner;
  DevBuf<unsigned long long> reqmask;
  DevBuf<double> leaf_sums;
  DevBuf<int> own_leaf;
  long long own_leaf_n = -1;
  int kept_rank = -1, kept_world = 0;
  std::vector<int> h_leaf_owner;
  std::vector<unsigned char> h_present;
  std::vector<double> h_node_sums;
  DevBuf<int> kept_row;
  std::vector<int64_t> kept_counts;
  long long kept_total = -1;
  DevBuf<double> kept_sums;
  DevBuf<double> leaf_len;
};

struct PmSlab
{
  int world = 0, rank = 0, N = 0, stage = -1;
  int xs = 0, nx = 0, ys = 0, ny = 0;
  int lo[3] = {0, 0, 0}, ext[3] = {0, 0, 0};
  int elo[3] = {0, 0, 0}, eext[3] = {0, 0, 0};
  std::vector<int> bbox;
  std::vector<int64_t> scount, rcount;
  long long edesc_off = 0;
  DevBuf<double> brick, slab, tbuf, ebrick, fmesh, send, recv;
  DevBuf<long long> desc;
  std::vector<long long> hdesc[2];
  int hdesc_turn = 0;
  void *plan2f = nullptr, *plan2i = nullptr, *plan1 = nullptr;
  int plan_N = 0, plan_nx = 0, plan_ny = 0;
  double bytes_sent[4] = {0, 0, 0, 0};
};

struct ngravs_ctx
{
  ngravs_config_t cfg;
  Tuning tune;
  PmSlab pms;
  TopTree top;
  DevBuf<int> n_top;
  ngravs_fatal_fn on_fatal = nullptr;
  hipStream_t stream = nullptr;
  double asmth = 0, rcut = 0;
  int64_t n = 0;
  int64_t n_local = 0;
  bool extent_override = false;
  double ext_lo[3], ext_hi[3];
  int dd_last_what = -1;
  long long dd_last_sent = 0;
  bool have_particles = false, have_order = false, have_tree = false, have_pm = false, have_acc = false;
  bool pm_parked = false;
  double dom[8] = {0, 0, 0, 0, 0, 0, 0, 0};
  double pos_lo[3] = {0, 0, 0}, pos_hi[3] = {-1, -1, -1};
  int64_t shard_first = 0, shard_count = 0;

  DevBuf<double> in_pos, in_mass, in_oldacc;
  DevBuf<double> in_cost;
  DevBuf<int> in_type;
  DevBuf<unsigned char> in_active;
  DevBuf<double2> in_rec;
  DevBuf<unsigned long long> in_key;
  DevBuf<long long> in_id;
  DevBuf<unsigned long long> dd_mask, dd_counts;
  int sort_low = 35;
  long long own_order_nlocal = -1, own_order_len = 0;
  DevBuf<unsigned char> dd_send, dd_recv;
  DevBuf<double4> s_pm;
  DevBuf<unsigned char> s_type, s_active;
  DevBuf<double> s_oldacc;
  DevBuf<unsigned long long> s_key;
  DevBuf<unsigned int> s_idx, idx_iota;
  DevBuf<unsigned char> sort_tmp;
  DevBuf<double> red_tmp;
  int64_t max_nodes = 0, nnodes = 0;
  bool tree_refit = false;
  bool tree_stale = false;
  int nlevels = 0;
  DevBuf<int> lvl_table;
  int lvl_table_level = 0;
  int64_t level_start[MAX_LEVELS + 2];
  DevBuf<int> n_first, n_count, n_child, n_flags, n_nchild;
  DevBuf<double4> n_geo, n_mom;
  DevBuf<int> tb_count;
  DevBuf<int> n_npart;
  DevBuf<int> scan_out;
  DevBuf<unsigned char> scan_tmp;
  DevBuf<int> d_counters;
  DevBuf<int> d_levels;
  long long level_hint[MAX_LEVELS + 2] = {0};
  DevBuf<double> table;
  bool table_ready = false;
  DevBuf<double> lat;
  bool lat_ready = false;
  DevBuf<int> walk_stack;
  DevBuf<int> walk_tlist;
  DevBuf<unsigned char> walk_tmp;
  long long walk_ntargets = -1;
  bool walk_dense_tlist = false;
  int walk_spread = 0;
  int walk_sg = 1;
  long long walk_unopened = 0;
  int walk_unit_state = 4;
  double walk_ia_ratio = 0;
  bool all_active = true;
  DevBuf<int> walk_ovf;
  DevBuf<int> walk_counters;
  DevBuf<double> r_acc, r_pm, r_oldacc;
  DevBuf<int> r_nint;
  int pm_plan_n = 0;
  void *fft_fwd = nullptr, *fft_inv = nullptr;
  DevBuf<double> pm_rho;
  DevBuf<double> pm_force;
  DevBuf<double> pm_phi;
  DevBuf<double> pm_orig;
  DevBuf<double> out_tmp;
  DevBuf<float> out_tmpf;
  std::vector<unsigned char> host_stage;
  ngravs_stats_t stats;
  hipEvent_t ev0 = nullptr, ev1 = nullptr, evk0 = nullptr, evk1 = nullptr;
  std::vector<hipEvent_t> ev_batch;
  int walk_batches = 0;
  int walk_lcap = 0;
  int walk_scap = 0;
  std::string last_error;
  std::vector<ngravs_user_fn_t> user_fns;
  std::vector<ngravs_user_lattice_t> user_lat;
  DevBuf<double> user_tab;
  UserTabs user_ut = {};
  bool user_ready = false;
  double user_soft[NGRAVS_NTYPES] = {0, 0, 0, 0, 0, 0};
  int last_walk_kernel = 0;
  hipStream_t pm_stream = nullptr, walk_stream = nullptr;
  int pm_stream_cus = 0;
  int device_cus = 0;
  int stream_cus = 0;
  int last_pm_cus = 0;
  double pm_solo_ms = 0, walk_solo_ms = 0;
  int pm_solo_steps = 0;
  int pm_auto_cus = -1;
  hipEvent_t ev_fork = nullptr, ev_pm0 = nullptr, ev_pm1 = nullptr, ev_walk = nullptr;
  DevBuf<int> probe_out;
  DevBuf<double> user_green;
  long long user_green_nk2 = 0;
  DevBuf<double> sph_vel_in, sph_h_in;
  DevBuf<double> sph_vel;
  DevBuf<int> sph_tlist;
  DevBuf<unsigned char> sph_tmp;
  DevBuf<double> sph_res;
  DevBuf<int> sph_row, sph_rounds;
  DevBuf<unsigned long long> sph_counters;
  DevBuf<double> sph_col_in;
  DevBuf<int> sph_ts_in;
  DevBuf<double> sph_hsrc;
  DevBuf<double> sph_hmax;
};

struct OnStream
{
  ngravs_ctx *c;
  hipStream_t s0;
  int n0;
  OnStream(ngravs_ctx *c_, hipStream_t s, int cus) : c(c_), s0(c_->stream), n0(c_->stream_cus)
  {
    c->stream = s;
    c->stream_cus = cus;
  }
  ~OnStream()
  {
    c->stream = s0;
    c->stream_cus = n0;
  }
};

int dom_find_extent(ngravs_ctx *c);
int dom_keys_and_sort(ngravs_ctx *c);
int dom_keys_only(ngravs_ctx *c, const double *d_pos, int64_t n, const double corner[3], double fac, int bits,
                  long long *d_keys);
int dd_local_extent(ngravs_ctx *c, double lo[3], double hi[3]);
void dd_apply_extent(ngravs_ctx *c, const double lo[3], const double hi[3]);
int dd_set_toptree(ngravs_ctx *c, int nnode, const int *child);
int dd_leaf_sums(ngravs_ctx *c, void **dev_sums, int64_t *count);
int dd_pack(ngravs_ctx *c, int what, const int *leaf_owner, int nranks, int me, int64_t *counts, void **dev_records, int64_t *nrec);
int dd_apply_migration(ngravs_ctx *c, const void *dev_records, int64_t nrec);
int dd_get_dest(ngravs_ctx *c, const int *leaf_owner, int *dest);
int dd_target_bounds(ngravs_ctx *c, double out[2]);
int dd_pack_leaves(ngravs_ctx *c, const unsigned long long *reqmask, int nranks, int me, int64_t *counts, void **dev_records, int64_t *nrec);
int dd_set_top(ngravs_ctx *c, const double *node_sums, const unsigned char *present);
int dd_set_halo(ngravs_ctx *c, const void *dev_records, int64_t nrec);
int dd_leaf_sums_kept(ngravs_ctx *c, void **dev_sums, int64_t *count);
int dd_pack_leaves_kept(ngravs_ctx *c, int64_t *counts, void **dev_records, int64_t *nrec);
int dd_refresh_halo(ngravs_ctx *c, const void *dev_records, int64_t nrec);
int dd_update_top(ngravs_ctx *c, const double *node_sums, const double *leaf_len);
int dd_peano_order_own(ngravs_ctx *c, int force);
int dd_fill_ids(ngravs_ctx *c);
int dd_record_doubles(const ngravs_ctx *c, int what);
int tree_build(ngravs_ctx *c);
int tree_moments(ngravs_ctx *c, bool refit, bool counts = false);
int tree_top_leaf_len(ngravs_ctx *c, double *dev_kept_sums, int stride);
int tree_top_refit(ngravs_ctx *c);
int dom_regather(ngravs_ctx *c);
static inline bool cfg_has_bam(const ngravs_config_t &cfg)
{
  for(int i = 0; i < cfg.n_gravs; i++)
    for(int j = 0; j < cfg.n_gravs; j++)
      if((cfg.law_accel[i][j] >= NGRAVS_LAW_BAMBAM && cfg.law_accel[i][j] < NGRAVS_LAW_USER0) ||
         (cfg.law_spline[i][j] >= NGRAVS_SPLINE_BAMBAM && cfg.law_spline[i][j] < NGRAVS_SPLINE_USER0))
        return true;
  return false;
}
static inline bool cfg_has_user(const ngravs_config_t &cfg)
{
  for(int i = 0; i < cfg.n_gravs; i++)
    for(int j = 0; j < cfg.n_gravs; j++)
      if(cfg.law_accel[i][j] >= NGRAVS_LAW_USER0 || cfg.law_spline[i][j] >= NGRAVS_SPLINE_USER0)
        return true;
  return false;
}
int user_check_config(const ngravs_config_t *cfg, const ngravs_user_fn_t *fns, int nfns, const ngravs_user_lattice_t *lat, int nlat,
                      std::string &why);
ngravs_lattice_fn user_lattice_fn(const ngravs_ctx *c, int a, int b);
bool user_lattice_complete(const ngravs_ctx *c);
int user_lattice_tabulate(ngravs_lattice_fn fn, double box, double *out, std::string &why);
void ngravs_report(ngravs_ctx *ctx, int code, const std::string &msg);
int user_tables_ensure(ngravs_ctx *c, double r_need);
int user_green_ensure(ngravs_ctx *c);
double user_normed(const ngravs_user_fn_t *fns, int nfns, int law, double k2);
void make_walk_params(const ngravs_ctx *c, WalkParams *wp);
int walk_run(ngravs_ctx *c);
int walk_finish(ngravs_ctx *c);
int direct_run(ngravs_ctx *c, const int *d_idx, int64_t nt, double *d_acc);
int direct_run_targets(ngravs_ctx *c, const double4 *d_tpm, const int *d_ttype, int64_t nt, double *d_acc, double r_need = 0);
int eval_ring_slots(const WalkParams &wp, bool yuk, int waves);
int launch_eval_ring(ngravs_ctx *c, const TreeView &tv, const WalkParams &wp, bool yuk, int nblk, int waves, int K, const int *region,
                     const int *gcount, long long g0, long long nb, int lcap, int scap, int S, const int *tlist, int SG, long long t_count);
#define SPH_KC1 2.546479089470
#define SPH_KC2 15.278874536822
#define SPH_KC3 45.836623610466
#define SPH_KC4 30.557749073644
#define SPH_KC5 5.092958178941
#define SPH_KC6 (-15.278874536822)
#define SPH_NORM_COEFF 4.188790204786
#define SPH_MAXITER 150
__host__ __device__ inline void sph_spline(double u, double hinv3, double hinv4, double *wk, double *dwk)
{
  if(u < 0.5)
    {
      *wk = hinv3 * (SPH_KC1 + SPH_KC2 * (u - 1) * u * u);
      *dwk = hinv4 * u * (SPH_KC3 * u - SPH_KC4);
    }
  else
    {
      *wk = hinv3 * SPH_KC5 * (1.0 - u) * (1.0 - u) * (1.0 - u);
      *dwk = hinv4 * SPH_KC6 * (1.0 - u) * (1.0 - u);
    }
}
enum { SPH_HSML = 0, SPH_DENSITY, SPH_NUMNGB, SPH_DIVVEL, SPH_CURLVEL, SPH_DHSML, SPH_NRES };
struct SphStats
{
  long long targets, bad_hsml, failed, stack_ovf, max_rounds, sum_rounds, candidates, neighbours;
};
int sph_density_run(ngravs_ctx *c, double des_num_ngb, double max_dev, double min_hsml, SphStats *st);
enum { SPH_HS_VX = 0, SPH_HS_VY, SPH_HS_VZ, SPH_HS_H, SPH_HS_RHO, SPH_HS_POR2, SPH_HS_CSJ, SPH_HS_F2, SPH_HS_TS, SPH_HS_CSI, SPH_HS_F1,
       SPH_HS_NCOL };
enum { SPH_HY_ACCX = 0, SPH_HY_ACCY, SPH_HY_ACCZ, SPH_HY_DTENTR, SPH_HY_MAXSIG, SPH_HY_NRES };
struct SphHydroParams
{
  int periodic, comoving, limiter, have_ts;
  double box, boxhalf;
  double hubble_a2, fac_mu, fac_vsic_fix;
  double visc, tbi, gamma;
};
struct SphHydroStats
{
  long long targets, bad_hsml, bad_density, bad_pressure, stack_ovf, candidates, pairs;
};
int sph_hydro_run(ngravs_ctx *c, const SphHydroParams &hp, SphHydroStats *st);
int sph_scatter(ngravs_ctx *c, const double *src, long long nt, double *dst, long long stride);
int pm_run(ngravs_ctx *c);
int pm_deposit(ngravs_ctx *c);
int pm_finish(ngravs_ctx *c);
void pm_release(ngravs_ctx *c);
int pmslab_begin(ngravs_ctx *c, int rank, int world, int bbox[6]);
int pmslab_pack(ngravs_ctx *c, int stage, const int *all_bbox, int64_t *send_counts, int64_t *recv_counts, void **send, void **recv);
int pmslab_unpack(ngravs_ctx *c, int stage);
void pmslab_release(ngravs_ctx *c);
void host_shortrange_table(const ngravs_config_t *cfg, double *force, double *pot, const ngravs_user_fn_t *fns = nullptr, int nfns = 0);
double cfg_asmth(const ngravs_config_t *c);
double cfg_rcut(const ngravs_config_t *c);
```

gadget-2.0.7-ngravs_amd/csrc/kernels_pm.hip:

```cpp
#include "engine.hpp"
#include "pm_common.hpp"
#include <hipfft/hipfft.h>

__global__ void k_cic_deposit(const double4 *__restrict__ s_pm, const unsigned char *__restrict__ s_type,
                              const unsigned char *__restrict__ s_flag, long long n,
                              double to_slab, int N, int ng, const int *__restrict__ t2g_tab, double *__restrict__ rho)
{
  long long i = blockIdx.x * (long long)blockDim.x + threadIdx.x;
  if(i >= n || (s_flag[i] & 2))
    return;
  double4 p = s_pm[i];
  int g = t2g_tab[s_type[i]];
  const long long NZ = N + 2;
  double *grid = rho + (size_t)g * N * N * NZ;
  double dx, dy, dz;
  int sx = cell_of(p.x, to_slab, N, &dx), sy = cell_of(p.y, to_slab, N, &dy), sz = cell_of(p.z, to_slab, N, &dz);
  int sxx = sx + 1 == N ? 0 : sx + 1, syy = sy + 1 == N ? 0 : sy + 1, szz = sz + 1 == N ? 0 : sz + 1;
  double m = p.w;
  atomicAdd(&grid[((long long)sx * N + sy) * NZ + sz], m * (1.0 - dx) * (1.0 - dy) * (1.0 - dz));
  atomicAdd(&grid[((long long)sx * N + syy) * NZ + sz], m * (1.0 - dx) * dy * (1.0 - dz));
  atomicAdd(&grid[((long long)sx * N + sy) * NZ + szz], m * (1.0 - dx) * (1.0 - dy) * dz);
  atomicAdd(&grid[((long long)sx * N + syy) * NZ + szz], m * (1.0 - dx) * dy * dz);
  atomicAdd(&grid[((long long)sxx * N + sy) * NZ + sz], m * (dx) * (1.0 - dy) * (1.0 - dz));
  atomicAdd(&grid[((long long)sxx * N + syy) * NZ + sz], m * (dx)*dy * (1.0 - dz));
  atomicAdd(&grid[((long long)sxx * N + sy) * NZ + szz], m * (dx) * (1.0 - dy) * dz);
  atomicAdd(&grid[((long long)sxx * N + syy) * NZ + szz], m * (dx)*dy * dz);
}

template <int NG>
__global__ void k_green(const double2 *__restrict__ rho, double2 *__restrict__ phi, GreenParams gp)
{
  const int N = gp.N, NH = N / 2 + 1;
  long long idx = blockIdx.x * (long long)blockDim.x + threadIdx.x;
  long long total = (long long)N * N * NH;
  if(idx >= total)
    return;
  int z = (int)(idx % NH);
  int y = (int)((idx / NH) % N);
  int x = (int)(idx / ((long long)NH * N));
  double2 out[NG];
  green_mode<NG>(gp, x, y, z, rho, (size_t)total, (size_t)idx, out);
#pragma unroll
  for(int b = 0; b < NG; b++)
    phi[(size_t)b * total + idx] = out[b];
}

__global__ void k_gradient_gather(const double4 *__restrict__ s_pm, const unsigned char *__restrict__ s_type,
                                  const unsigned char *__restrict__ s_flag,
                                  long long first, long long n, double to_slab, int N, const int *__restrict__ t2g_tab,
                                  const double *__restrict__ phi, double fac, double *__restrict__ r_pm)
{
  long long i = blockIdx.x * (long long)blockDim.x + threadIdx.x;
  if(i >= n)
    return;
  i += first;
  if(s_flag[i] & 2)
    {
      r_pm[3 * i + 0] = r_pm[3 * i + 1] = r_pm[3 * i + 2] = 0.0;
      return;
    }
  double4 p = s_pm[i];
  int g = t2g_tab[s_type[i]];
  const long long NZ = N + 2;
  const double *grid = phi + (size_t)g * N * N * NZ;
  double dx, dy, dz;
  int sx = cell_of(p.x, to_slab, N, &dx), sy = cell_of(p.y, to_slab, N, &dy), sz = cell_of(p.z, to_slab, N, &dz);
  double wx[2] = {1.0 - dx, dx}, wy[2] = {1.0 - dy, dy}, wz[2] = {1.0 - dz, dz};
  double acc[3] = {0, 0, 0};
  auto wrap = [N](int a) { return a < 0 ? a + N : (a >= N ? a - N : a); };
  auto at = [&](int x, int y, int z) { return grid[((long long)x * N + y) * NZ + z]; };
  const int ox[8] = {0, 0, 0, 0, 1, 1, 1, 1}, oy[8] = {0, 1, 0, 1, 0, 1, 0, 1}, oz[8] = {0, 0, 1, 1, 0, 0, 1, 1};
  for(int c = 0; c < 8; c++)
    {
      int x = wrap(sx + ox[c]), y = wrap(sy + oy[c]), z = wrap(sz + oz[c]);
      double w = wx[ox[c]] * wy[oy[c]] * wz[oz[c]];
      double fxv = fac * ((4.0 / 3) * (at(wrap(x - 1), y, z) - at(wrap(x + 1), y, z)) -
                          (1.0 / 6) * (at(wrap(x - 2), y, z) - at(wrap(x + 2), y, z)));
      double fyv = fac * ((4.0 / 3) * (at(x, wrap(y - 1), z) - at(x, wrap(y + 1), z)) -
                          (1.0 / 6) * (at(x, wrap(y - 2), z) - at(x, wrap(y + 2), z)));
      double fzv = fac * ((4.0 / 3) * (at(x, y, wrap(z - 1)) - at(x, y, wrap(z + 1))) -
                          (1.0 / 6) * (at(x, y, wrap(z - 2)) - at(x, y, wrap(z + 2))));
      acc[0] += fxv * w;
      acc[1] += fyv * w;
      acc[2] += fzv * w;
    }
  r_pm[3 * i + 0] = acc[0];
  r_pm[3 * i + 1] = acc[1];
  r_pm[3 * i + 2] = acc[2];
}

#define FM_XB 64
__global__ __launch_bounds__(256) void k_force_mesh_march(const double *__restrict__ grid, int N, double fac, double *__restrict__ fm)
{
  const long long NZ = N + 2;
  const int z = blockIdx.x * 32 + (threadIdx.x & 31), y = blockIdx.y * 8 + (threadIdx.x >> 5);
  const int x0 = blockIdx.z * FM_XB;
  if(z >= N || y >= N)
    return;
  auto wrap = [N](int a) { return a < 0 ? a + N : (a >= N ? a - N : a); };
  const int ym1 = wrap(y - 1), yp1 = wrap(y + 1), ym2 = wrap(y - 2), yp2 = wrap(y + 2);
  const int zm1 = wrap(z - 1), zp1 = wrap(z + 1), zm2 = wrap(z - 2), zp2 = wrap(z + 2);
  auto at = [&](int xx, int yy, int zz) { return grid[((long long)xx * N + yy) * NZ + zz]; };
  double pm2 = at(wrap(x0 - 2), y, z), pm1 = at(wrap(x0 - 1), y, z), p0 = at(wrap(x0), y, z), pp1 = at(wrap(x0 + 1), y, z);
  const int x1 = x0 + FM_XB < N ? x0 + FM_XB : N;
  __shared__ double stage[4][2][96];
  const int wave = threadIdx.x >> 6, lane = threadIdx.x & 63, zl = threadIdx.x & 31, rw = (threadIdx.x >> 5) & 1;
  const bool full = blockIdx.x * 32 + 32 <= N && blockIdx.y * 8 + 8 <= N && (N % 2) == 0;
  for(int x = x0; x < x1; x++)
    {
      const double pp2 = at(wrap(x + 2), y, z);
      const double fy = fac * ((4.0 / 3) * (at(x, ym1, z) - at(x, yp1, z)) - (1.0 / 6) * (at(x, ym2, z) - at(x, yp2, z)));
      const double fz = fac * ((4.0 / 3) * (at(x, y, zm1) - at(x, y, zp1)) - (1.0 / 6) * (at(x, y, zm2) - at(x, y, zp2)));
      const double fx = fac * ((4.0 / 3) * (pm1 - pp1) - (1.0 / 6) * (pm2 - pp2));
      const long long idx = ((long long)x * N + y) * N + z;
      if(full)
        {
          stage[wave][rw][3 * zl + 0] = fx;
          stage[wave][rw][3 * zl + 1] = fy;
          stage[wave][rw][3 * zl + 2] = fz;
          __builtin_amdgcn_fence(__ATOMIC_SEQ_CST, "wavefront");
          __builtin_amdgcn_wave_barrier();
          const int yw = blockIdx.y * 8 + 2 * wave;
#pragma unroll
          for(int q = lane; q < 96; q += 64)
            {
              const int r = q / 48, o = q - 48 * r;
              const double2 v = *reinterpret_cast<const double2 *>(&stage[wave][r][2 * o]);
              *reinterpret_cast<double2 *>(fm + 3 * (((long long)x * N + yw + r) * N + blockIdx.x * 32) + 2 * o) = v;
            }
          __builtin_amdgcn_fence(__ATOMIC_SEQ_CST, "wavefront");
          __builtin_amdgcn_wave_barrier();
        }
      else
        {
          fm[3 * idx + 0] = fx;
          fm[3 * idx + 1] = fy;
          fm[3 * idx + 2] = fz;
        }
      pm2 = pm1;
      pm1 = p0;
      p0 = pp1;
      pp1 = pp2;
    }
}

__global__ void k_gather_force(const double4 *__restrict__ s_pm, const unsigned char *__restrict__ s_type,
                               const unsigned char *__restrict__ s_flag, long long first, long long n, double to_slab, int N,
                               const int *__restrict__ t2g_tab, int species, const double *__restrict__ fm,
                               double *__restrict__ r_pm)
{
  long long i = blockIdx.x * (long long)blockDim.x + threadIdx.x;
  if(i >= n)
    return;
  i += first;
  if(s_flag[i] & 2)
    {
      if(species <= 0)
        r_pm[3 * i + 0] = r_pm[3 * i + 1] = r_pm[3 * i + 2] = 0.0;
      return;
    }
  const int g = t2g_tab[s_type[i]];
  if(species >= 0 && g != species)
    return;
  if(species < 0)
    fm += (size_t)g * 3 * N * N * N;
  const double4 p = s_pm[i];
  double dx, dy, dz;
  int sx = cell_of(p.x, to_slab, N, &dx), sy = cell_of(p.y, to_slab, N, &dy), sz = cell_of(p.z, to_slab, N, &dz);
  double wx[2] = {1.0 - dx, dx}, wy[2] = {1.0 - dy, dy}, wz[2] = {1.0 - dz, dz};
  double acc[3] = {0, 0, 0};
  auto wrap = [N](int a) { return a < 0 ? a + N : (a >= N ? a - N : a); };
  typedef double d2u __attribute__((ext_vector_type(2), aligned(8)));
  const int z1 = wrap(sz + 1);
  const bool zpair = z1 == sz + 1;
  double fv[8][3];
#pragma unroll
  for(int cx = 0; cx < 2; cx++)
#pragma unroll
    for(int cy = 0; cy < 2; cy++)
      {
        const int x = wrap(sx + cx), y = wrap(sy + cy);
        const double *f0 = fm + 3 * (((long long)x * N + y) * N + sz);
        const int c0 = 4 * cx + cy, c1 = 4 * cx + cy + 2;
        if(zpair)
          {
            const d2u a = *reinterpret_cast<const d2u *>(f0), b_ = *reinterpret_cast<const d2u *>(f0 + 2),
                      c_ = *reinterpret_cast<const d2u *>(f0 + 4);
            fv[c0][0] = a.x;
            fv[c0][1] = a.y;
            fv[c0][2] = b_.x;
            fv[c1][0] = b_.y;
            fv[c1][1] = c_.x;
            fv[c1][2] = c_.y;
          }
        else
          {
            const double *f1 = fm + 3 * (((long long)x * N + y) * N + z1);
#pragma unroll
            for(int d = 0; d < 3; d++)
              {
                fv[c0][d] = f0[d];
                fv[c1][d] = f1[d];
              }
          }
      }
  const int ox[8] = {0, 0, 0, 0, 1, 1, 1, 1}, oy[8] = {0, 1, 0, 1, 0, 1, 0, 1}, oz[8] = {0, 0, 1, 1, 0, 0, 1, 1};
#pragma unroll
  for(int c = 0; c < 8; c++)
    {
      const double w = wx[ox[c]] * wy[oy[c]] * wz[oz[c]];
      acc[0] += fv[c][0] * w;
      acc[1] += fv[c][1] * w;
      acc[2] += fv[c][2] * w;
    }
  r_pm[3 * i + 0] = acc[0];
  r_pm[3 * i + 1] = acc[1];
  r_pm[3 * i + 2] = acc[2];
}

#define PM_DT 18
#define PM_TILE_THREADS 1024


template <int NG>
__global__ __launch_bounds__(PM_TILE_THREADS) void k_cic_deposit_tiled(
    const double4 *__restrict__ s_pm, const unsigned char *__restrict__ s_type, const unsigned char *__restrict__ s_flag,
    const int *__restrict__ n_first, const int *__restrict__ n_count, const double4 *__restrict__ n_geo, int node0,
    double to_slab, int N, const int *__restrict__ t2g_tab, double *__restrict__ rho, MeshAddr ma)
{
  constexpr int DT = PM_DT;
  extern __shared__ double tile[];
  const int node = node0 + blockIdx.x;
  const double4 geo = n_geo[node];
  const int first = n_first[node], count = n_count[node];
  int o[3];
  {
    const double h = 0.5 * geo.w;
    o[0] = (int)floor((geo.x - h) * to_slab);
    o[1] = (int)floor((geo.y - h) * to_slab);
    o[2] = (int)floor((geo.z - h) * to_slab);
  }
  for(int t = threadIdx.x; t < NG * DT * DT * DT; t += blockDim.x)
    tile[t] = 0.0;
  __syncthreads();
  for(int k = threadIdx.x; k < count; k += blockDim.x)
    {
      const int i = first + k;
      if(s_flag[i] & 2)
        continue;
      const double4 p = s_pm[i];
      const int g = t2g_tab[s_type[i]];
      double dx, dy, dz;
      const int sx = cell_of(p.x, to_slab, N, &dx), sy = cell_of(p.y, to_slab, N, &dy), sz = cell_of(p.z, to_slab, N, &dz);
      const int lx = sx - o[0], ly = sy - o[1], lz = sz - o[2];
      const double m = p.w;
      const double w[8] = {m * (1.0 - dx) * (1.0 - dy) * (1.0 - dz), m * (1.0 - dx) * dy * (1.0 - dz),
                           m * (1.0 - dx) * (1.0 - dy) * dz,         m * (1.0 - dx) * dy * dz,
                           m * (dx) * (1.0 - dy) * (1.0 - dz),       m * (dx)*dy * (1.0 - dz),
                           m * (dx) * (1.0 - dy) * dz,               m * (dx)*dy * dz};
      const int ox[8] = {0, 0, 0, 0, 1, 1, 1, 1}, oy[8] = {0, 1, 0, 1, 0, 1, 0, 1}, oz[8] = {0, 0, 1, 1, 0, 0, 1, 1};
      if(lx >= 0 && ly >= 0 && lz >= 0 && lx < DT - 1 && ly < DT - 1 && lz < DT - 1)
        {
          double *tg = tile + (size_t)g * DT * DT * DT;
#pragma unroll
          for(int c = 0; c < 8; c++)
            atomicAdd(&tg[((lx + ox[c]) * DT + (ly + oy[c])) * DT + (lz + oz[c])], w[c]);
        }
      else
        {
          double *grid = rho + (size_t)g * ma.species_stride();
#pragma unroll
          for(int c = 0; c < 8; c++)
            atomicAdd(&grid[ma.cell(sx + ox[c], sy + oy[c], sz + oz[c])], w[c]);
        }
    }
  __syncthreads();
  for(int t = threadIdx.x; t < NG * DT * DT * DT; t += blockDim.x)
    {
      const double v = tile[t];
      if(v != 0.0)
        {
          const int g = t / (DT * DT * DT), r = t % (DT * DT * DT);
          const int lx = r / (DT * DT), ly = (r / DT) % DT, lz = r % DT;
          atomicAdd(&rho[(size_t)g * ma.species_stride() + ma.cell(o[0] + lx, o[1] + ly, o[2] + lz)], v);
        }
    }
}

__global__ void k_cic_deposit_loose(const double4 *__restrict__ s_pm, const unsigned char *__restrict__ s_type,
                                    const unsigned char *__restrict__ s_flag,
                                    const int *__restrict__ n_child, int nnodes_above, double to_slab, int N,
                                    const int *__restrict__ t2g_tab, double *__restrict__ rho, MeshAddr ma)
{
  long long t = blockIdx.x * (long long)blockDim.x + threadIdx.x;
  if(t >= 8ll * nnodes_above)
    return;
  const int c = n_child[t];
  if(c > -2)
    return;
  const int i = -2 - c;
  if(s_flag[i] & 2)
    return;
  double4 p = s_pm[i];
  int g = t2g_tab[s_type[i]];
  double *grid = rho + (size_t)g * ma.species_stride();
  double dx, dy, dz;
  int sx = cell_of(p.x, to_slab, N, &dx), sy = cell_of(p.y, to_slab, N, &dy), sz = cell_of(p.z, to_slab, N, &dz);
  double m = p.w;
  atomicAdd(&grid[ma.cell(sx, sy, sz)], m * (1.0 - dx) * (1.0 - dy) * (1.0 - dz));
  atomicAdd(&grid[ma.cell(sx, sy + 1, sz)], m * (1.0 - dx) * dy * (1.0 - dz));
  atomicAdd(&grid[ma.cell(sx, sy, sz + 1)], m * (1.0 - dx) * (1.0 - dy) * dz);
  atomicAdd(&grid[ma.cell(sx, sy + 1, sz + 1)], m * (1.0 - dx) * dy * dz);
  atomicAdd(&grid[ma.cell(sx + 1, sy, sz)], m * (dx) * (1.0 - dy) * (1.0 - dz));
  atomicAdd(&grid[ma.cell(sx + 1, sy + 1, sz)], m * (dx)*dy * (1.0 - dz));
  atomicAdd(&grid[ma.cell(sx + 1, sy, sz + 1)], m * (dx) * (1.0 - dy) * dz);
  atomicAdd(&grid[ma.cell(sx + 1, sy + 1, sz + 1)], m * (dx)*dy * dz);
}

static int pm_tile_level(const ngravs_ctx *c, double to_slab)
{
  if(!c->have_tree)
    return -1;
  double len = c->dom[6];
  for(int l = 0; l < c->nlevels && l < TREE_BITS; l++, len *= 0.5)
    if(len * to_slab <= 16.0 * 1.002)
      return (c->level_start[l + 1] - c->level_start[l] > 0) ? l : -1;
  return -1;
}

void pm_release(ngravs_ctx *c)
{
  if(c->fft_fwd)
    {
      hipfftDestroy(*(hipfftHandle *)c->fft_fwd);
      delete(hipfftHandle *)c->fft_fwd;
      c->fft_fwd = nullptr;
    }
  if(c->fft_inv)
    {
      hipfftDestroy(*(hipfftHandle *)c->fft_inv);
      delete(hipfftHandle *)c->fft_inv;
      c->fft_inv = nullptr;
    }
  c->pm_plan_n = 0;
}

int pm_deposit_tiles(ngravs_ctx *c, const MeshAddr &ma, double *dst)
{
  const int N = c->cfg.pmgrid, ng = c->cfg.n_gravs;
  const double to_slab = N / c->cfg.box_size;
  const int bs = 256;
  const int tl = pm_tile_level(c, to_slab);
  if(tl < 0)
    return 1;
  const long long tl0 = c->level_start[tl], tln = c->level_start[tl + 1] - tl0;
  const size_t lds = sizeof(double) * ng * PM_DT * PM_DT * PM_DT;
  auto launch_dep = [&](auto kern) -> int {
    HIP_TRY(c, hipFuncSetAttribute(reinterpret_cast<const void *>(kern), hipFuncAttributeMaxDynamicSharedMemorySize, (int)lds));
    hipLaunchKernelGGL(kern, dim3((unsigned)tln), dim3(PM_TILE_THREADS), lds, c->stream, c->s_pm.p, c->s_type.p, c->s_active.p,
                       c->n_first.p, c->n_count.p, c->n_geo.p, (int)tl0, to_slab, N, c->d_counters.p + 8, dst, ma);
    return NGRAVS_OK;
  };
  const int rc = ng == 1 ? launch_dep(k_cic_deposit_tiled<1>) : (ng == 2 ? launch_dep(k_cic_deposit_tiled<2>) : launch_dep(k_cic_deposit_tiled<3>));
  if(rc)
    return rc;
  if(tl0 > 0)
    hipLaunchKernelGGL(k_cic_deposit_loose, dim3((unsigned)((8 * tl0 + bs - 1) / bs)), dim3(bs), 0, c->stream, c->s_pm.p, c->s_type.p,
                       c->s_active.p, c->n_child.p, (int)tl0, to_slab, N, c->d_counters.p + 8, dst, ma);
  HIP_TRY(c, hipGetLastError());
  return NGRAVS_OK;
}

int pm_deposit(ngravs_ctx *c)
{
  const int N = c->cfg.pmgrid, ng = c->cfg.n_gravs;
  const long long n = c->n;
  if(N <= 0 || !c->cfg.periodic)
    {
      ngravs_report(c, NGRAVS_ERR_ARG, "pmforce_periodic needs PERIODIC and PMGRID");
      return NGRAVS_ERR_ARG;
    }
  const size_t real_elems = (size_t)N * N * (N + 2);
  if(c->pm_rho.ensure(real_elems * ng) || c->pm_phi.ensure(real_elems * ng) || c->r_pm.ensure(3 * n) || c->d_counters.ensure(16))
    return NGRAVS_ERR_NOMEM;
  if(c->pm_plan_n != N)
    {
      pm_release(c);
      c->fft_fwd = new hipfftHandle;
      c->fft_inv = new hipfftHandle;
      FFT_TRY(c, hipfftPlan3d((hipfftHandle *)c->fft_fwd, N, N, N, HIPFFT_D2Z));
      FFT_TRY(c, hipfftPlan3d((hipfftHandle *)c->fft_inv, N, N, N, HIPFFT_Z2D));
      c->pm_plan_n = N;
    }
  FFT_TRY(c, hipfftSetStream(*(hipfftHandle *)c->fft_fwd, c->stream));
  FFT_TRY(c, hipfftSetStream(*(hipfftHandle *)c->fft_inv, c->stream));
  HIP_TRY(c, hipMemcpyAsync(c->d_counters.p + 8, c->cfg.type_to_grav, sizeof(int) * 6, hipMemcpyHostToDevice, c->stream));
  const double L = c->cfg.box_size, to_slab = N / L;
  HIP_TRY(c, hipMemsetAsync(c->pm_rho.p, 0, sizeof(double) * real_elems * ng, c->stream));
  const int bs = 256;
  unsigned nbp = (unsigned)((n + bs - 1) / bs);
  MeshAddr ma;
  ma.N = N;
  ma.brick = 0;
  for(int j = 0; j < 3; j++)
    {
      ma.lo[j] = 0;
      ma.ext[j] = N;
    }
  int rct = pm_deposit_tiles(c, ma, c->pm_rho.p);
  if(rct == 1)
    hipLaunchKernelGGL(k_cic_deposit, dim3(nbp), dim3(bs), 0, c->stream, c->s_pm.p, c->s_type.p, c->s_active.p, n, to_slab, N, ng,
                       c->d_counters.p + 8, c->pm_rho.p);
  else if(rct)
    return rct;
  HIP_TRY(c, hipGetLastError());
  return NGRAVS_OK;
}

int pm_finish(ngravs_ctx *c)
{
  const int N = c->cfg.pmgrid, ng = c->cfg.n_gravs;
  const long long n = c->n;
  const size_t real_elems = (size_t)N * N * (N + 2);
  const double L = c->cfg.box_size, to_slab = N / L;
  const int bs = 256;
  for(int a = 0; a < ng; a++)
    FFT_TRY(c, hipfftExecD2Z(*(hipfftHandle *)c->fft_fwd, c->pm_rho.p + real_elems * a,
                             (hipfftDoubleComplex *)(c->pm_rho.p + real_elems * a)));
  int rcg = user_green_ensure(c);
  if(rcg)
    return rcg;
  GreenParams gp;
  make_green_params(c, &gp);
  long long modes = (long long)N * N * (N / 2 + 1);
  unsigned nbm = (unsigned)((modes + bs - 1) / bs);
  switch(ng)
    {
    case 1:
      hipLaunchKernelGGL(k_green<1>, dim3(nbm), dim3(bs), 0, c->stream, (const double2 *)c->pm_rho.p, (double2 *)c->pm_phi.p, gp);
      break;
    case 2:
      hipLaunchKernelGGL(k_green<2>, dim3(nbm), dim3(bs), 0, c->stream, (const double2 *)c->pm_rho.p, (double2 *)c->pm_phi.p, gp);
      break;
    default:
      hipLaunchKernelGGL(k_green<3>, dim3(nbm), dim3(bs), 0, c->stream, (const double2 *)c->pm_rho.p, (double2 *)c->pm_phi.p, gp);
      break;
    }
  for(int b = 0; b < ng; b++)
    FFT_TRY(c, hipfftExecZ2D(*(hipfftHandle *)c->fft_inv, (hipfftDoubleComplex *)(c->pm_phi.p + real_elems * b),
                             c->pm_phi.p + real_elems * b));
  double fac = c->cfg.G / (M_PI * L);
  fac *= 1 / (2 * L / N);
  if(c->cfg.world_size > 1)
    HIP_TRY(c, hipMemsetAsync(c->r_pm.p, 0, sizeof(double) * 3 * n, c->stream));
  unsigned nbg = (unsigned)((c->shard_count + bs - 1) / bs);
  if(nbg > 0 && c->cfg.world_size <= 2)
    {
      const long long NN = (long long)N * N * N;
      const size_t fm_all = (size_t)3 * NN * ng * sizeof(double), fm_have = c->pm_force.cap * sizeof(double);
      size_t free_b = 0, total_b = 0;
      bool all_resident = fm_all <= ((size_t)16 << 30) || fm_have >= fm_all;
      if(!all_resident && hipMemGetInfo(&free_b, &total_b) == hipSuccess)
        all_resident = free_b + fm_have >= fm_all + ((size_t)48 << 30);
      if(c->pm_force.ensure((size_t)(3 * NN) * (all_resident ? ng : 1)))
        return NGRAVS_ERR_NOMEM;
      if(all_resident)
        {
          for(int b = 0; b < ng; b++)
            hipLaunchKernelGGL(k_force_mesh_march, dim3((N + 31) / 32, (N + 7) / 8, (N + FM_XB - 1) / FM_XB), dim3(256), 0, c->stream,
                               c->pm_phi.p + real_elems * b, N, fac, c->pm_force.p + (size_t)3 * NN * b);
          hipLaunchKernelGGL(k_gather_force, dim3(nbg), dim3(bs), 0, c->stream, c->s_pm.p, c->s_type.p, c->s_active.p,
                             (long long)c->shard_first, (long long)c->shard_count, to_slab, N, c->d_counters.p + 8, -1, c->pm_force.p,
                             c->r_pm.p);
        }
      else
      for(int b = 0; b < ng; b++)
        {
          hipLaunchKernelGGL(k_force_mesh_march, dim3((N + 31) / 32, (N + 7) / 8, (N + FM_XB - 1) / FM_XB), dim3(256), 0, c->stream,
                             c->pm_phi.p + real_elems * b, N, fac, c->pm_force.p);
          hipLaunchKernelGGL(k_gather_force, dim3(nbg), dim3(bs), 0, c->stream, c->s_pm.p, c->s_type.p, c->s_active.p,
                             (long long)c->shard_first, (long long)c->shard_count, to_slab, N, c->d_counters.p + 8, b, c->pm_force.p,
                             c->r_pm.p);
        }
    }
  else if(nbg > 0)
    hipLaunchKernelGGL(k_gradient_gather, dim3(nbg), dim3(bs), 0, c->stream, c->s_pm.p, c->s_type.p, c->s_active.p, (long long)c->shard_first,
                       (long long)c->shard_count, to_slab, N, c->d_counters.p + 8, c->pm_phi.p, fac, c->r_pm.p);
  HIP_TRY(c, hipGetLastError());
  c->have_pm = true;
  return NGRAVS_OK;
}

int pm_run(ngravs_ctx *c)
{
  int rc = pm_deposit(c);
  if(rc)
    return rc;
  return pm_finish(c);
}
```

gadget-2.0.7-ngravs_amd/csrc/kernels_walk.hip:

```cpp
#include "engine.hpp"
#include "walk_device.hpp"
#include "eval_asm.inc"
#include <hipcub/hipcub.hpp>
#include <type_traits>

__device__ __forceinline__ double bam_eta(int law, double target, double m, double N, double eps)
{
  if(law == NGRAVS_LAW_BAMBAM)
    return 4.0 * M_PI * eps / (target + m / N);
  if(law == NGRAVS_LAW_SOURCEBAM)
    return 4.0 * M_PI * eps * N / m;
  return 4.0 * M_PI * eps / target;
}
__device__ __forceinline__ double bam_accel(int law, double target, double m, double r, double N, double eps)
{
  double eta = bam_eta(law, target, m, N, eps), rho = 2 * target * m / M_PI;
  double reta = r * eta, reta2 = reta * reta, eta3 = eta * eta * eta;
  if(reta < 0.1)
    return rho * eta3 * (2.0 * r / 3.0 - 4.0 * reta2 * r / 5.0 + 6.0 * reta2 * reta2 * r / 7.0);
  return rho * eta3 * (atan(reta) / (reta2 * eta) - 1.0 / (reta * eta * (1 + reta2)));
}
__device__ __forceinline__ double bam_spline(int law, double target, double m, double r, double N, double eps)
{
  double eta = bam_eta(law, target, m, N, eps), rho = 2 * target * m / M_PI;
// ... 2182 lines not shown
  size_t bytes;
};
static EvalLds eval_lds(const WalkParams &wp, bool tables, int max_waves)
{
  const size_t fixed = (tables ? sizeof(double) * (wp.ntab_lds + wp.exp_tab) * NTAB : 0) + 40 * sizeof(double);
  int waves = (int)((160 * 1024 - fixed) / GW2_WAVE_LDS);
  if(waves > max_waves)
    waves = max_waves;
  if(waves < 1)
    waves = 1;
  return {waves, fixed + (size_t)waves * GW2_WAVE_LDS};
}

template <int NG, int PM, int YUK, int TAB_LDS, int LATT, int USR>
static int launch_group2_t(Row<NG, PM, YUK, TAB_LDS, LATT, USR>, ngravs_ctx *c, const WalkParams &wp, int *glist, int nlist)
{
  const int S0 = c->walk_spread > 1 ? c->walk_spread : 1, G0 = (WAVE / S0) * (glist ? c->walk_sg : 1);
  int S = S0;
  if(glist)
    {
      const int want = nlist <= 4096 ? 64 : (nlist <= 65536 ? 8 : 1);
      S = want > S0 ? want : S0;
    }
  const int G = WAVE / S;
  const int ncu = walk_cus(c);
  const EvalLds l = eval_lds(wp, PM && TAB_LDS, GW_MAXWAVES);
  const int waves = l.waves;
  const size_t lds = l.bytes;
  long long ngroups = glist ? (long long)nlist * (G0 / G) : (walk_tcount(c) + G - 1) / G;
  long long nblk = ncu;
  if(nblk > (ngroups + waves - 1) / waves)
    nblk = (ngroups + waves - 1) / waves;
  if(nblk < 1)
    nblk = 1;
  if(c->walk_stack.ensure((size_t)nblk * waves * (GW_STACK + (size_t)NG * GW2_ITEMS)) || c->walk_counters.ensure(32))
    return NGRAVS_ERR_NOMEM;
  if(glist)
    HIP_TRY(c, hipMemsetAsync(c->walk_counters.p + 8, 0, sizeof(int) * 8, c->stream));
  else
    HIP_TRY(c, hipMemsetAsync(c->walk_counters.p, 0, sizeof(int) * 32, c->stream));
  auto kern = k_walk_group2<NG, PM, YUK, TAB_LDS, LATT, 0, USR>;
  HIP_TRY(c, hipFuncSetAttribute(reinterpret_cast<const void *>(kern), hipFuncAttributeMaxDynamicSharedMemorySize, (int)lds));
  hipLaunchKernelGGL(kern, dim3((unsigned)nblk), dim3(waves * 64), lds, c->stream, tree_view(c), c->s_pm.p,
                     c->s_type.p, c->s_oldacc.p, c->s_active.p, LATT ? c->lat.p : c->table.p, wp, (long long)c->shard_first,
                     walk_tcount(c), c->walk_counters.p, c->walk_stack.p, c->walk_counters.p + 1, c->r_acc.p,
                     c->r_nint.p, (int *)nullptr, (int *)nullptr, 0ll, glist ? (long long)nlist : 0ll, 0, 0, glist, S, G0, walk_tlist(c), 1);
  return NGRAVS_OK;
}

static int walk_unit_next(int st, double r)
{
  if(!(r > 0))
    return st;
  if(st == 4)
    return r > 2.0 ? 1 : (r > 1.4 ? 2 : 4);
  if(st == 2)
    return r > 2.0 ? 1 : (r < 1.2 ? 4 : 2);
  return r < 1.2 ? 4 : (r < 1.7 ? 2 : 1);
}

template <int NG, int PM, int YUK, int TAB_LDS, int LATT, int USR>
static int launch_group3_t(Row<NG, PM, YUK, TAB_LDS, LATT, USR>, ngravs_ctx *c, const WalkParams &wp)
{
  const int ncu = walk_cus(c);
  const int max_waves = c->tune.walk_waves > 0 && c->tune.walk_waves < GW2_MAXWAVES ? c->tune.walk_waves : GW2_MAXWAVES;
  const EvalLds l = eval_lds(wp, PM && TAB_LDS, max_waves);
  int waves = l.waves;
  const size_t lds = l.bytes;
  const int S = c->walk_spread > 1 ? c->walk_spread : 1, G = WAVE / S;
  const long long ngroups = (walk_tcount(c) + G - 1) / G;
  int SG = (PM && (c->walk_ntargets < 0 || c->walk_dense_tlist)) ? 4 : 1;
  if(SG == 4)
    SG = c->walk_unit_state = walk_unit_next(c->walk_unit_state, c->walk_ia_ratio);
  if(c->tune.walk_sg >= 1)
    SG = c->tune.walk_sg;
  if(SG != c->walk_sg)
    c->walk_lcap = 0;
  c->walk_sg = SG;
  const long long nunits = (ngroups + SG - 1) / SG;
  if(c->walk_lcap < 1024)
    {
      c->walk_lcap = (NG == 1 ? 2 : 1) * (SG > 1 ? 2 : 1) * GW3_LIST_MIN;
      if(c->tune.walk_lcap >= 1024)
        c->walk_lcap = c->tune.walk_lcap;
    }
  if(c->walk_scap < GW3_STK_MIN)
    c->walk_scap = GW3_STK_MIN;
  c->walk_lcap &= ~3;
  const int lcap = c->walk_lcap, scap = c->walk_scap;
  const size_t region_ints = (size_t)NG * lcap + scap;
  long long batch = 1 << 20;
  size_t cap_bytes = (size_t)8 << 30;
  {
    size_t free_b = 0, total_b = 0;
    if(hipMemGetInfo(&free_b, &total_b) == hipSuccess)
      {
        free_b += c->walk_stack.cap * sizeof(int);
        if(free_b / 4 > cap_bytes)
          cap_bytes = free_b / 4;
        if(cap_bytes > ((size_t)64 << 30))
          cap_bytes = (size_t)64 << 30;
      }
  }
  if(c->tune.walk_batch > 0)
    {
      batch = c->tune.walk_batch;
      cap_bytes = (size_t)64 << 30;
    }
  while(batch > 8192 && (size_t)batch * region_ints * sizeof(int) > cap_bytes)
    batch /= 2;
  if(batch > nunits)
    batch = nunits;
  if(batch < 1)
    batch = 1;
  if(c->walk_stack.ensure((size_t)batch * (region_ints + NG + 2)) || c->walk_counters.ensure(32) ||
     c->walk_ovf.ensure((size_t)nunits))
    return NGRAVS_ERR_NOMEM;
  int *region = c->walk_stack.p, *gcount = c->walk_stack.p + (size_t)batch * region_ints;
  HIP_TRY(c, hipMemsetAsync(c->walk_counters.p, 0, sizeof(int) * 32, c->stream));
  auto kt = k_walk_group2<NG, PM, YUK, TAB_LDS, LATT, 1, USR>;
  auto ke = k_walk_group2<NG, PM, YUK, TAB_LDS, LATT, 2, USR>;
  HIP_TRY(c, hipFuncSetAttribute(reinterpret_cast<const void *>(ke), hipFuncAttributeMaxDynamicSharedMemorySize, (int)lds));
  int ringK = 0, ring_waves = waves;
  if constexpr(PM && TAB_LDS && !LATT && !USR)
    if(c->tune.walk_ring)
      {
        ring_waves = max_waves;
        ringK = eval_ring_slots(wp, YUK, ring_waves);
        if(c->tune.walk_ring_k >= 4 && c->tune.walk_ring_k < ringK)
          ringK = c->tune.walk_ring_k;
        if(ringK)
          waves = ring_waves;
      }
  const size_t nbatches = (size_t)((nunits + batch - 1) / batch);
  while(c->ev_batch.size() < 3 * nbatches)
    {
      hipEvent_t e;
      HIP_TRY(c, hipEventCreate(&e));
      c->ev_batch.push_back(e);
    }
  c->walk_batches = (int)nbatches;
  size_t ib = 0;
  for(long long u0 = 0; u0 < nunits; u0 += batch, ib++)
    {
      const long long nbu = nunits - u0 < batch ? nunits - u0 : batch;
      const long long g0 = u0 * SG, nb = ngroups - g0 < nbu * SG ? ngroups - g0 : nbu * SG;
      HIP_TRY(c, hipEventRecord(c->ev_batch[3 * ib], c->stream));
      const long long tblk = 8 * (((nbu + GW3_TBLOCK / 64 - 1) / (GW3_TBLOCK / 64) + 7) / 8);
      hipLaunchKernelGGL(kt, dim3((unsigned)tblk), dim3(GW3_TBLOCK), 0, c->stream, tree_view(c), c->s_pm.p, c->s_type.p,
                         c->s_oldacc.p, c->s_active.p, LATT ? c->lat.p : c->table.p, wp, (long long)c->shard_first,
                         walk_tcount(c), c->walk_counters.p, (int *)nullptr, c->walk_counters.p + 1, c->r_acc.p,
                         c->r_nint.p, region, gcount, u0, nbu, lcap, scap, c->walk_ovf.p, S, G, walk_tlist(c), SG);
      HIP_TRY(c, hipEventRecord(c->ev_batch[3 * ib + 1], c->stream));
      if(g0 > 0)
        HIP_TRY(c, hipMemsetAsync(c->walk_counters.p + 8, 0, sizeof(int) * 8, c->stream));
      long long nblk = ncu;
      if(nblk > (nb + waves - 1) / waves)
        nblk = (nb + waves - 1) / waves;
      if(ringK)
        {
          int rr = launch_eval_ring(c, tree_view(c), wp, YUK, (int)nblk, ring_waves, ringK, region, gcount, g0, nb, lcap, scap, S,
                                    walk_tlist(c), SG, walk_tcount(c));
          if(rr != NGRAVS_OK)
            return rr;
        }
      else
      hipLaunchKernelGGL(ke, dim3((unsigned)nblk), dim3(waves * 64), lds, c->stream, tree_view(c), c->s_pm.p, c->s_type.p,
                         c->s_oldacc.p, c->s_active.p, LATT ? c->lat.p : c->table.p, wp, (long long)c->shard_first,
                         walk_tcount(c), c->walk_counters.p, (int *)nullptr, c->walk_counters.p + 1, c->r_acc.p,
                         c->r_nint.p, region, gcount, g0, nb, lcap, scap, c->walk_ovf.p, S, G, walk_tlist(c), SG);
      HIP_TRY(c, hipEventRecord(c->ev_batch[3 * ib + 2], c->stream));
    }
  return NGRAVS_OK;
}

struct GroupVariant
{
  bool pm, yuk, tab, latt, usr;
  int reports;
};
static GroupVariant group_variant(const ngravs_ctx *c, const WalkParams &wp, int ng)
{
  const bool yuk = has_yukawa(c), usr = wp.user != 0;
  const int id = usr ? NGRAVS_KERNEL_GROUP_USER : NGRAVS_KERNEL_GROUP;
  if(c->cfg.pmgrid)
    {
      const bool tab = ng <= 2 || (!usr && wp.ntab_lds + wp.exp_tab <= 3);
      return {true, yuk && !usr, tab, false, usr, id};
    }
  if(c->cfg.periodic)
    return {false, yuk && !usr, false, true, usr, id};
  const bool bam = wp.bam && (!yuk || usr);
  return {false, yuk && !bam, bam, false, false, bam ? id : NGRAVS_KERNEL_GROUP};
}
template <int NG>
using GroupRowsNG = Table<Row<NG, 1, 0, NG <= 2, 0, 1>, Row<NG, 1, 0, NG <= 2, 0, 0>, Row<NG, 1, 1, NG <= 2, 0, 0>,
                          Row<NG, 1, 0, 1, 0, 0>, Row<NG, 1, 1, 1, 0, 0>,
                          Row<NG, 0, 0, 0, 1, 1>, Row<NG, 0, 0, 0, 1, 0>, Row<NG, 0, 1, 0, 1, 0>,
                          Row<NG, 0, 0, 1, 0, 0>, Row<NG, 0, 0, 0, 0, 0>, Row<NG, 0, 1, 0, 0, 0>>;
using GroupRows = decltype(GroupRowsNG<1>{} + GroupRowsNG<2>{} + GroupRowsNG<3>{});

static int launch_group(ngravs_ctx *c, const WalkParams &wp, bool *used_split, int *glist = nullptr, int nlist = 0)
{
  const bool split = !c->tune.walk_fused && !glist;
  if(!glist)
    {
      c->walk_batches = 0;
      *used_split = split;
    }
  const GroupVariant v = group_variant(c, wp, c->cfg.n_gravs);
  c->last_walk_kernel = v.reports;
  const int key[] = {c->cfg.n_gravs, v.pm, v.yuk, v.tab, v.latt, v.usr};
  return dispatch(c, GroupRows{}, key, [&](auto row) {
    if(split)
      return launch_group3_t(row, c, wp);
    return launch_group2_t(row, c, wp, glist, nlist);
  });
}

static double user_reach(const ngravs_ctx *c) { return c->cfg.pmgrid ? 1.25 * 6.0 * c->asmth : 1.25 * sqrt(3.0) * c->dom[6]; }
static double lattice_reach(const ngravs_ctx *c) { return 1.25 * 0.5 * sqrt(3.0) * c->cfg.box_size; }

static int walk_spread_choice(const ngravs_ctx *c, const WalkParams &wp, bool latt)
{
  const bool pm = c->cfg.pmgrid != 0;
  const int tuned = c->tune.walk_spread;
  if(c->walk_ntargets >= 0 && !c->walk_dense_tlist && pm && c->cfg.box_size > 0)
    {
      if(tuned >= 1)
        return tuned > 1 ? tuned : 0;
      const double vol_per_target = pow(c->cfg.box_size, 3) * (double)c->shard_count / ((double)c->n * (double)(c->walk_ntargets > 0 ? c->walk_ntargets : 1));
      return cbrt(vol_per_target * 64.0) > 2.5 * sqrt(wp.reach2) ? 64 : 0;
    }
  if(tuned > 1)
    return tuned;
  if(tuned == 0)
    {
      const long long g64 = (walk_tcount(c) + WAVE - 1) / WAVE;
      if(pm && c->walk_unit_state == 1 && c->walk_ia_ratio > 2.0)
        return 2;
      if(!pm && !latt && g64 > 0 && g64 < 2048)
        return g64 < 1024 ? 4 : 2;
    }
  return 0;
}

static int walk_read_back(ngravs_ctx *c, int *flag, unsigned long long (&st64)[4])
{
  HIP_TRY(c, hipMemcpyAsync(flag, c->walk_counters.p + 1, sizeof(int), hipMemcpyDeviceToHost, c->stream));
  HIP_TRY(c, hipMemcpyAsync(st64, c->walk_counters.p + 16, 4 * sizeof(unsigned long long), hipMemcpyDeviceToHost, c->stream));
  HIP_TRY(c, hipStreamSynchronize(c->stream));
  return NGRAVS_OK;
}

int walk_run(ngravs_ctx *c)
{
  const long long n = c->n;
  if(c->r_acc.ensure(3 * n) || c->r_nint.ensure(n) || c->r_oldacc.ensure(n))
    return NGRAVS_ERR_NOMEM;
  const bool latt = c->cfg.periodic && !c->cfg.pmgrid;
  if(latt)
    {
      int rcl = ensure_lattice(c);
      if(rcl)
        return rcl;
    }
  {
    int rcu = user_tables_ensure(c, latt ? lattice_reach(c) : user_reach(c));
    if(rcu)
      return rcu;
  }
  WalkParams wp;
  make_walk_params(c, &wp);
  LawIds li;
  make_law_ids(c, &li);
  c->walk_ntargets = -1;
  const bool strict = c->cfg.walk_mode == NGRAVS_WALK_STRICT;
  if(c->top.on && c->cfg.pmgrid)
    {
      const double need = strict ? 6.0 : fmin(6.0, c->cfg.group_reach > 0 ? c->cfg.group_reach : NGRAVS_GROUP_REACH);
      if(need > c->top.import_reach * (1.0 + 1e-12))
        {
          ngravs_report(c, NGRAVS_ERR_STATE, "the walk reaches farther than the multi-task decomposition imported for: set the walk mode "
                                             "(and group_reach) before the decomposition");
          return NGRAVS_ERR_STATE;
        }
    }
  if(!strict)
    {
      int rct = ensure_level_table(c, sqrt(wp.reach2));
      if(rct)
        return rct;
      if((rct = walk_select_targets(c)))
        return rct;
    }
  if(!(c->all_active && c->cfg.world_size == 1 && c->n_local == c->n))
    {
      HIP_TRY(c, hipMemsetAsync(c->r_nint.p, 0, sizeof(int) * n, c->stream));
      HIP_TRY(c, hipMemsetAsync(c->r_acc.p, 0, sizeof(double) * 3 * n, c->stream));
      HIP_TRY(c, hipMemcpyAsync(c->r_oldacc.p, c->s_oldacc.p, sizeof(double) * n, hipMemcpyDeviceToDevice, c->stream));
    }
  const bool pm = c->cfg.pmgrid != 0;
  HIP_TRY(c, hipEventRecord(c->evk0, c->stream));
  int rc = NGRAVS_OK;
  bool used_split = false;
  if(strict)
// ... 147 lines not shown
```

include/ngravs_hip.h:

```cpp
#ifndef NGRAVS_HIP_H
#define NGRAVS_HIP_H

#include <stdint.h>
#include <stddef.h>

#ifdef __cplusplus
extern "C" {
#endif

#define NGRAVS_ABI_VERSION 3
#define NGRAVS_MAX_GRAVS 3
#define NGRAVS_NTYPES 6
#define NGRAVS_NTAB 2048
#define NGRAVS_ASMTH 1.25
#define NGRAVS_RCUT 4.5
#define NGRAVS_BITS_PER_DIMENSION 18
#define NGRAVS_GROUP_REACH 4.5
#define NGRAVS_TREE_BITS 21

typedef enum {
  NGRAVS_LAW_NONE = 0,
  NGRAVS_LAW_NEWTON = 1,
  NGRAVS_LAW_NEG_NEWTON = 2,
  NGRAVS_LAW_YUKAWA = 3,
  NGRAVS_LAW_COLOYUK = 4,
  NGRAVS_LAW_BAMBAM = 5,
  NGRAVS_LAW_SOURCEBAM = 6,
  NGRAVS_LAW_TARGETBAM = 7,
  NGRAVS_LAW_COUNT
} ngravs_law;

typedef enum {
  NGRAVS_SPLINE_NONE = 0,
  NGRAVS_SPLINE_PLUMMER = 1,
  NGRAVS_SPLINE_NEG_PLUMMER = 2,
  NGRAVS_SPLINE_BAMBAM = 3,
  NGRAVS_SPLINE_SOURCEBAM = 4,
  NGRAVS_SPLINE_TARGETBAM = 5,
  NGRAVS_SPLINE_COUNT
} ngravs_spline;

#define NGRAVS_LAW_USER0 64
#define NGRAVS_SPLINE_USER0 64
#define NGRAVS_MAX_USER_FNS 8

typedef enum {
  NGRAVS_OK = 0,
  NGRAVS_ERR_ARG = -1,
  NGRAVS_ERR_NO_DEVICE = -2,
  NGRAVS_ERR_NOMEM = -3,
  NGRAVS_ERR_STATE = -4,
  NGRAVS_ERR_TREE = -5,
  NGRAVS_ERR_WIRING = -6
} ngravs_status;

typedef enum {
  NGRAVS_WALK_STRICT = 0,
  NGRAVS_WALK_GROUP = 1
} ngravs_walk_mode;

typedef struct {
  int32_t abi_version;
  int32_t n_gravs;
  int32_t periodic;
  int32_t pmgrid;
  double box_size;
  double G;
  double err_tol_theta;
  double err_tol_force_acc;
  double force_softening[NGRAVS_NTYPES];
  int32_t type_to_grav[NGRAVS_NTYPES];
  int32_t law_accel[NGRAVS_MAX_GRAVS][NGRAVS_MAX_GRAVS];
  int32_t law_spline[NGRAVS_MAX_GRAVS][NGRAVS_MAX_GRAVS];
  int32_t law_greens[NGRAVS_MAX_GRAVS][NGRAVS_MAX_GRAVS];
  int32_t law_normed[NGRAVS_MAX_GRAVS][NGRAVS_MAX_GRAVS];
  double yukawa_imass;
  double asmth;
  double rcut;
  double tree_alloc_factor;
  double group_reach;
  int32_t walk_mode;
  int32_t device;
  int32_t rank, world_size;
  double bam_epsilon;
  int32_t reserved[6];
} ngravs_config_t;

typedef struct {
  int64_t n;
  const double *pos;           int64_t pos_stride;
  const double *mass;          int64_t mass_stride;
  const int32_t *type;         int64_t type_stride;
  const double *old_acc;      int64_t old_acc_stride;
  const uint8_t *active;
  int64_t active_stride;
  const double *grav_pm;
  int64_t grav_pm_stride;
  const float *grav_cost;
  int64_t grav_cost_stride;
  int32_t on_device;
  int32_t reserved;
} ngravs_particles_t;

typedef struct {
  int64_t n_active;
  int64_t n_nodes;
  double interactions;
  double t_domain, t_peano, t_treebuild, t_treewalk, t_pm;
  double walk_kernel_ms;
  double reserved[7];
} ngravs_stats_t;

typedef struct ngravs_ctx ngravs_ctx;
typedef void (*ngravs_fatal_fn)(int code, const char *msg);

typedef double (*ngravs_gravity_fn)(double, double, double, double, long);
typedef enum {
  NGRAVS_USER_ACCEL = 0,
  NGRAVS_USER_SPLINE = 1,
  NGRAVS_USER_GREENS = 2,
  NGRAVS_USER_NORMED = 3
} ngravs_user_kind;
typedef struct {
  int32_t kind;
  int32_t reserved;
  ngravs_gravity_fn fn;
} ngravs_user_fn_t;
typedef void (*ngravs_lattice_fn)(int i, int j, int k, double x[3], double force[3]);
typedef struct {
  int32_t target, source;
  ngravs_lattice_fn fn;
} ngravs_user_lattice_t;
typedef enum {
  NGRAVS_KERNEL_NONE = 0,
  NGRAVS_KERNEL_STRICT = 1,
  NGRAVS_KERNEL_STRICT_USER = 2,
  NGRAVS_KERNEL_GROUP = 3,
  NGRAVS_KERNEL_GROUP_USER = 4
} ngravs_walk_kernel_id;

int ngravs_abi_version(void);
const char *ngravs_build_info(void);
void ngravs_config_default(ngravs_config_t *cfg);
int ngravs_create(const ngravs_config_t *cfg, ngravs_ctx **out);
int ngravs_create_with_laws(const ngravs_config_t *cfg, const ngravs_user_fn_t *fns, int nfns, ngravs_ctx **out);
int ngravs_create_with_lattice(const ngravs_config_t *cfg, const ngravs_user_fn_t *fns, int nfns, const ngravs_user_lattice_t *lat,
                               int nlat, ngravs_ctx **out);
int ngravs_last_walk_kernel(ngravs_ctx *ctx);
int ngravs_last_pm_cus(ngravs_ctx *ctx);
int ngravs_cu_probe(ngravs_ctx *ctx, int which, int nblocks, int32_t *cu_ids);
void ngravs_destroy(ngravs_ctx *ctx);
void ngravs_set_fatal_handler(ngravs_ctx *ctx, ngravs_fatal_fn fn);
int ngravs_set_opening(ngravs_ctx *ctx, double err_tol_theta, double err_tol_force_acc);
int ngravs_set_walk_mode(ngravs_ctx *ctx, int walk_mode);
int ngravs_set_softening(ngravs_ctx *ctx, const double force_softening[NGRAVS_NTYPES]);
int ngravs_get_config(ngravs_ctx *ctx, ngravs_config_t *out);
int ngravs_set_tuning(ngravs_ctx *ctx, const char *name, double value);
int ngravs_memcpy(ngravs_ctx *ctx, void *dst, const void *src, int64_t bytes, int kind);
int ngravs_device_alloc(ngravs_ctx *ctx, void **ptr, int64_t bytes);
int ngravs_device_free(ngravs_ctx *ctx, void *ptr);

int ngravs_set_particles(ngravs_ctx *ctx, const ngravs_particles_t *p);
int ngravs_update_particles(ngravs_ctx *ctx, const ngravs_particles_t *p);
int ngravs_set_old_acc(ngravs_ctx *ctx, const double *old_acc, int64_t stride, int on_device);

int ngravs_domain_decomposition(ngravs_ctx *ctx);
int ngravs_discard_grav_pm(ngravs_ctx *ctx);
int64_t ngravs_force_treebuild(ngravs_ctx *ctx);
int ngravs_force_update_tree(ngravs_ctx *ctx);
int ngravs_gravity_tree(ngravs_ctx *ctx);
int ngravs_pmforce_periodic(ngravs_ctx *ctx);
int ngravs_compute_accelerations(ngravs_ctx *ctx, int pm_step);

int ngravs_get_accel(ngravs_ctx *ctx, double *grav_accel, int64_t accel_stride,
                     double *grav_pm, int64_t pm_stride, double *old_acc, int64_t old_acc_stride,
                     float *grav_cost, int64_t cost_stride, int on_device, int only_active);
int ngravs_get_stats(ngravs_ctx *ctx, ngravs_stats_t *out);
int ngravs_walk_unopened(ngravs_ctx *ctx, int64_t *count);
int ngravs_get_domain(ngravs_ctx *ctx, double out[8]);
int ngravs_get_keys(ngravs_ctx *ctx, int64_t *keys, int on_device);
int ngravs_get_order(ngravs_ctx *ctx, int32_t *order, int on_device);
int ngravs_get_shard(ngravs_ctx *ctx, int64_t *first, int64_t *count);
const char *ngravs_last_error(ngravs_ctx *ctx);

int64_t ngravs_peano_hilbert_key(int x, int y, int z, int bits);
int ngravs_peano_keys(ngravs_ctx *ctx, const double *pos, int64_t n, const double corner[3],
                      double fac, int bits, int64_t *keys);
int ngravs_shortrange_table(const ngravs_config_t *cfg, double *force_out, double *pot_out);
int ngravs_shortrange_table_with_laws(const ngravs_config_t *cfg, const ngravs_user_fn_t *fns, int nfns, double *force_out,
                                      double *pot_out);
int ngravs_user_table_eval(const ngravs_user_fn_t *fn, double r_lo, double r_hi, double h, const double *r, int64_t n, double *out,
                           double *max_err);
int ngravs_user_lattice_table(ngravs_lattice_fn fn, double box_size, double *out);
int ngravs_direct_sum(ngravs_ctx *ctx, const int32_t *idx, int64_t nt, double *acc);
int ngravs_direct_sum_targets(ngravs_ctx *ctx, const double *pos, const double *mass, const int32_t *type, int64_t nt, double *acc);

#define NGRAVS_DD_RECORD_BYTES 56
#define NGRAVS_DD_MAX_RECORD_BYTES 80
int64_t ngravs_dd_record_bytes(ngravs_ctx *ctx, int what);
int64_t ngravs_dd_num_local(ngravs_ctx *ctx);
int ngravs_dd_local_extent(ngravs_ctx *ctx, double lo[3], double hi[3]);
int ngravs_dd_peano_order(ngravs_ctx *ctx, int force);
int ngravs_dd_set_extent(ngravs_ctx *ctx, const double lo[3], const double hi[3]);
int ngravs_get_domain_extent(ngravs_ctx *ctx, double out[8]);
int ngravs_dd_set_toptree(ngravs_ctx *ctx, int32_t nnode, const int32_t *child);
int ngravs_dd_get_toptree(ngravs_ctx *ctx, int32_t *nnode, const int32_t **child);
#define NGRAVS_TOP_CW(ng) (7 + 4 * (ng))
int ngravs_dd_leaf_sums(ngravs_ctx *ctx, void **dev_sums, int64_t *count);
int ngravs_dd_target_bounds(ngravs_ctx *ctx, double out[2]);
int ngravs_dd_keep_margin(ngravs_ctx *ctx, double *margin);
int ngravs_dd_pack(ngravs_ctx *ctx, int what, const int32_t *leaf_owner, int nranks, int my_rank, int64_t *counts, void **dev_records,
                   int64_t *nrec);
int ngravs_dd_get_dest(ngravs_ctx *ctx, const int32_t *leaf_owner, int32_t *dest);
int ngravs_dd_pack_leaves(ngravs_ctx *ctx, const uint64_t *reqmask, int nranks, int my_rank, int64_t *counts, void **dev_records,
                          int64_t *nrec);
int ngravs_dd_set_top(ngravs_ctx *ctx, const double *node_sums, const uint8_t *present);
int ngravs_dd_recv_buffer(ngravs_ctx *ctx, int64_t nrec, void **dev_records);
int ngravs_dd_apply_migration(ngravs_ctx *ctx, const void *dev_records, int64_t nrec);
int ngravs_dd_set_halo(ngravs_ctx *ctx, const void *dev_records, int64_t nrec);
int ngravs_dd_leaf_sums_kept(ngravs_ctx *ctx, void **dev_sums, int64_t *count);
int ngravs_dd_pack_leaves_kept(ngravs_ctx *ctx, int64_t *counts, void **dev_records, int64_t *nrec);
int ngravs_dd_refresh_halo(ngravs_ctx *ctx, const void *dev_records, int64_t nrec);
int ngravs_dd_update_top(ngravs_ctx *ctx, const double *node_sums, const double *leaf_len);
int ngravs_dd_get_kept(ngravs_ctx *ctx, int32_t *rank, int32_t *world, const int32_t **leaf_owner, const uint8_t **present,
                       const double **node_sums);
int ngravs_dd_set_ids(ngravs_ctx *ctx, const int64_t *ids, int on_device);
int ngravs_dd_get_ids(ngravs_ctx *ctx, int64_t *ids, int on_device);
int ngravs_pm_slab_begin(ngravs_ctx *ctx, int rank, int world, int32_t bbox[6]);
int ngravs_pm_slab_pack(ngravs_ctx *ctx, int stage, const int32_t *all_bbox, int64_t *send_counts, int64_t *recv_counts,
                        void **send, void **recv);
int ngravs_pm_slab_unpack(ngravs_ctx *ctx, int stage);
int ngravs_pm_slab_bytes(ngravs_ctx *ctx, double bytes[4]);

typedef struct {
  const double *vel_pred; int64_t vel_stride;
  double *hsml;           int64_t hsml_stride;
  double des_num_ngb, max_num_ngb_deviation, min_gas_hsml;
  int32_t on_device, reserved;
} ngravs_sph_in_t;
typedef struct {
  double *density, *num_ngb, *div_vel, *curl_vel, *dhsml_factor;
  int64_t density_stride, num_ngb_stride, div_vel_stride, curl_vel_stride, dhsml_factor_stride;
} ngravs_sph_out_t;
int ngravs_sph_density(ngravs_ctx *ctx, const ngravs_sph_in_t *in, const ngravs_sph_out_t *out, int32_t *max_rounds,
                       double *kernel_ms);
int ngravs_sph_kernel(double h, const double *r, int64_t n, double *wk, double *dwk);

typedef struct {
  const double *vel_pred;     int64_t vel_pred_stride;
  const double *hsml;         int64_t hsml_stride;
  const double *density;      int64_t density_stride;
  const double *pressure;     int64_t pressure_stride;
  const double *dhsml_factor; int64_t dhsml_factor_stride;
  const double *div_vel;      int64_t div_vel_stride;
  const double *curl_vel;     int64_t curl_vel_stride;
  const int32_t *timestep;    int64_t timestep_stride;
  double art_bulk_visc_const, timebase_interval, gamma;
  double hubble_a2, fac_mu, fac_vsic_fix;
  int32_t viscosity_limiter, comoving, on_device, reserved;
} ngravs_hydro_in_t;
typedef struct {
  double *hydro_accel, *dt_entropy, *max_signal_vel;
  int64_t hydro_accel_stride, dt_entropy_stride, max_signal_vel_stride;
} ngravs_hydro_out_t;
int ngravs_sph_hydro(ngravs_ctx *ctx, const ngravs_hydro_in_t *in, const ngravs_hydro_out_t *out, double *kernel_ms);

#ifdef __cplusplus
}
#endif
#endif
```

Measured before the change: 624.1 million.

## Start PM deposit from Peano keys on a separate stream before tree build

```diff
diff --git a/gadget-2.0.7-ngravs_amd/__init__.py b/gadget-2.0.7-ngravs_amd/__init__.py
--- a/gadget-2.0.7-ngravs_amd/__init__.py
+++ b/gadget-2.0.7-ngravs_amd/__init__.py
@@ -14,7 +14,7 @@
 
 EXPORTS = [
     "ngravs_abi_version", "ngravs_build_info", "ngravs_config_default", "ngravs_create", "ngravs_create_with_laws", "ngravs_destroy",
-    "ngravs_last_walk_kernel", "ngravs_last_pm_cus", "ngravs_cu_probe", "ngravs_shortrange_table_with_laws", "ngravs_user_table_eval",
+    "ngravs_last_walk_kernel", "ngravs_last_pm_cus", "ngravs_last_pm_early", "ngravs_pm_patch_table", "ngravs_cu_probe", "ngravs_shortrange_table_with_laws", "ngravs_user_table_eval",
     "ngravs_create_with_lattice", "ngravs_user_lattice_table",
     "ngravs_set_fatal_handler", "ngravs_set_opening", "ngravs_set_walk_mode", "ngravs_set_softening", "ngravs_dd_record_bytes", "ngravs_get_config", "ngravs_set_tuning",
     "ngravs_memcpy", "ngravs_device_alloc", "ngravs_device_free",
@@ -108,6 +108,9 @@
         L.ngravs_last_walk_kernel.argtypes = [C.c_void_p]
         L.ngravs_last_pm_cus.argtypes = [C.c_void_p]
         L.ngravs_cu_probe.argtypes = [C.c_void_p, C.c_int, C.c_int, C.c_void_p]
+        L.ngravs_last_pm_early.argtypes = [C.c_void_p, C.c_void_p]
+        L.ngravs_pm_patch_table.restype = C.c_int64
+        L.ngravs_pm_patch_table.argtypes = [C.c_void_p, C.c_int, C.c_int64, C.c_void_p, C.c_void_p, C.c_void_p, C.c_void_p]
         L.ngravs_shortrange_table_with_laws.argtypes = [C.c_void_p, C.c_void_p, C.c_int, C.c_void_p, C.c_void_p]
         L.ngravs_user_table_eval.argtypes = [C.c_void_p, C.c_double, C.c_double, C.c_double, C.c_void_p, C.c_int64, C.c_void_p,
                                              C.c_void_p]
@@ -219,6 +222,21 @@
 
     def last_pm_cus(self):
         return int(lib().ngravs_last_pm_cus(self._h))
+
+    def last_pm_early(self):
+        ph = np.zeros(3)
+        return int(lib().ngravs_last_pm_early(self._h, ph.ctypes.data)), ph
+
+    def pm_patch_table(self, from_tree):
+        nl = C.c_int64(0)
+        n = int(lib().ngravs_pm_patch_table(self._h, int(from_tree), 1 << 30, None, None, None, None))
+        if n < 0:
+            self._check(n, "ngravs_pm_patch_table")
+        first, count, geo = np.zeros(n, np.int32), np.zeros(n, np.int32), np.zeros((n, 4))
+        n2 = int(lib().ngravs_pm_patch_table(self._h, int(from_tree), n, first.ctypes.data, count.ctypes.data, geo.ctypes.data, C.byref(nl)))
+        if n2 != n:
+            self._check(min(n2, -1), "ngravs_pm_patch_table")
+        return first, count, geo, int(nl.value)
 
     def cu_probe(self, which, nblocks=2048):
         out = np.zeros(nblocks, dtype=np.int32)
diff --git a/gadget-2.0.7-ngravs_amd/csrc/capi.hip b/gadget-2.0.7-ngravs_amd/csrc/capi.hip
--- a/gadget-2.0.7-ngravs_amd/csrc/capi.hip
+++ b/gadget-2.0.7-ngravs_amd/csrc/capi.hip
@@ -411,6 +411,17 @@
       (void)hipStreamDestroy(c->pm_stream);
       (void)hipStreamDestroy(c->walk_stream);
     }
+  if(c->early_stream)
+    {
+      (void)hipStreamSynchronize(c->early_stream);
+      (void)hipStreamDestroy(c->early_stream);
+    }
+  c->pmk_cell.release();
+  c->pmk_first.release();
+  c->pmk_count.release();
+  c->pmk_n.release();
+  c->pmk_geo.release();
+  c->pmk_tmp.release();
   c->probe_out.release();
   (void)hipStreamDestroy(c->stream);
   delete c;
@@ -507,6 +518,8 @@
     t.tree_levelwise = iv != 0;
   else if(k == "dd_keep" && v >= 0 && v <= 0.25)
     t.dd_keep = v;
+  else if(k == "pm_early" && (iv == -1 || iv == 0 || iv == 1))
+    t.pm_early = (int)iv;
   else if(k == "pm_cus" && (iv == -1 || (iv >= 0 && iv <= 32 && iv % 8 == 0)))
     t.pm_cus = (int)iv;
   else if(k == "sph_verbose")
@@ -599,7 +612,7 @@
       c->sort_low = 35;
       c->all_active = true;
       c->walk_ia_ratio = 0;
-      c->pm_solo_steps = 0, c->pm_auto_cus = -1;
+      c->pm_solo_steps = 0, c->pm_auto_cus = -1, c->pm_early_state = -1;
       c->walk_unit_state = 4;
       c->have_particles = true;
       c->have_order = c->have_tree = c->have_pm = c->have_acc = false;
@@ -721,7 +734,7 @@
     hipLaunchKernelGGL(k_fill_u8, GRID1(n), 0, c->stream, c->in_active.p, (long long)n, (unsigned char)1);
   HIP_TRY(c, hipGetLastError());
   c->walk_ia_ratio = 0;
-  c->pm_solo_steps = 0, c->pm_auto_cus = -1;
+  c->pm_solo_steps = 0, c->pm_auto_cus = -1, c->pm_early_state = -1;
   c->walk_unit_state = 4;
   c->have_particles = true;
   if(keep_tree)
@@ -983,7 +996,13 @@
          c->n > 0 && c->n_local > 0;
 }
 
-static int gravity_tree_impl(ngravs_ctx *c, hipEvent_t pm_done)
+struct EvalWait
+{
+  ngravs_ctx *c;
+  EvalWait(ngravs_ctx *c_, hipEvent_t e) : c(c_) { c->eval_wait = e; }
+  ~EvalWait() { c->eval_wait = nullptr; }
+};
+static int gravity_tree_impl(ngravs_ctx *c, hipEvent_t pm_done, bool early = false)
 {
   if(!c || !c->have_order)
     return NGRAVS_ERR_STATE;
@@ -1009,7 +1028,7 @@
       return NGRAVS_OK;
     }
   HIP_TRY(c, hipEventRecord(c->ev0, c->stream));
-  const bool masked = (pm_done || (c->tune.pm_cus > 0 && overlap_eligible(c))) && masked_streams(c, pm_done ? c->pm_stream_cus : c->tune.pm_cus) == NGRAVS_OK;
+  const bool masked = !early && (pm_done || (c->tune.pm_cus > 0 && overlap_eligible(c))) && masked_streams(c, pm_done ? c->pm_stream_cus : c->tune.pm_cus) == NGRAVS_OK;
   if(masked)
     {
       HIP_TRY(c, hipStreamWaitEvent(c->walk_stream, c->ev0, 0));
@@ -1021,8 +1040,12 @@
       HIP_TRY(c, hipEventRecord(c->ev_walk, c->walk_stream));
       HIP_TRY(c, hipStreamWaitEvent(c->stream, c->ev_walk, 0));
     }
-  else if((rc = walk_run(c)))
-    return rc;
+  else
+    {
+      EvalWait w(c, early ? pm_done : nullptr);
+      if((rc = walk_run(c)))
+        return rc;
+    }
   if(pm_done)
     HIP_TRY(c, hipStreamWaitEvent(c->stream, pm_done, 0));
   if((rc = walk_finish(c)))
@@ -1060,11 +1083,11 @@
 
 extern "C" int ngravs_gravity_tree(ngravs_ctx *c) { return gravity_tree_impl(c, nullptr); }
 
-static int pm_on_masked_stream(ngravs_ctx *c)
+static int pm_on_stream(ngravs_ctx *c, hipStream_t s, int cus)
 {
   HIP_TRY(c, hipEventRecord(c->ev_fork, c->stream));
-  HIP_TRY(c, hipStreamWaitEvent(c->pm_stream, c->ev_fork, 0));
-  OnStream on(c, c->pm_stream, c->pm_stream_cus);
+  HIP_TRY(c, hipStreamWaitEvent(s, c->ev_fork, 0));
+  OnStream on(c, s, cus);
   HIP_TRY(c, hipEventRecord(c->ev_pm0, c->stream));
   int rc = pm_run(c);
   if(rc)
@@ -1081,17 +1104,17 @@
   int rc;
   if(!c->have_order && (rc = ngravs_domain_decomposition(c)))
     return rc;
-  if(!c->have_tree)
+  if(c->have_tree && c->tree_stale && (rc = ngravs_force_update_tree(c)))
+    return rc;
+  if(!pm_keys_describe_tree(c) && !c->have_tree)
     {
       int64_t nn = ngravs_force_treebuild(c);
       if(nn < 0)
         return (int)nn;
     }
-  else if(c->tree_stale && (rc = ngravs_force_update_tree(c)))
-    return rc;
   if(c->tune.pm_cus > 0 && overlap_eligible(c) && masked_streams(c, c->tune.pm_cus) == NGRAVS_OK)
     {
-      if((rc = pm_on_masked_stream(c)))
+      if((rc = pm_on_stream(c, c->pm_stream, c->pm_stream_cus)))
         return rc;
       float ms = 0;
       HIP_TRY(c, hipEventSynchronize(c->ev_pm1));
@@ -1134,6 +1157,47 @@
   return c->pm_auto_cus;
 }
 
+static const double PM_EARLY_FIT = 1.5;
+static bool choose_pm_early(ngravs_ctx *c)
+{
+  if(!overlap_eligible(c) || c->tune.pm_early == 0)
+    return false;
+  if(c->tune.pm_early == 1)
+    return true;
+  if(c->tune.pm_cus >= 0 || c->tune.walk_fused)
+    return false;
+  if(c->pm_early_state < 0 && c->pm_solo_steps >= 2 && c->pm_solo_ms > 0 && c->build_solo_ms + c->trav_solo_ms > 0)
+    c->pm_early_state = c->pm_solo_ms <= PM_EARLY_FIT * (c->build_solo_ms + c->trav_solo_ms) ? 1 : 0;
+  return c->pm_early_state == 1;
+}
+
+static int early_step(ngravs_ctx *c)
+{
+  if(!c->early_stream)
+    HIP_TRY(c, hipStreamCreate(&c->early_stream));
+  int rc;
+  if((rc = pm_on_stream(c, c->early_stream, 0)))
+    return rc;
+  int64_t nn = ngravs_force_treebuild(c);
+  if(nn < 0)
+    return (int)nn;
+  if((rc = gravity_tree_impl(c, c->ev_pm1, true)))
+    return rc;
+  float ms = 0, t_pm = 0, t_trav = 0;
+  (void)hipEventElapsedTime(&ms, c->ev_pm0, c->ev_pm1);
+  c->stats.t_pm = ms * 1e-3;
+  (void)hipEventElapsedTime(&t_pm, c->ev_fork, c->ev_pm1);
+  if(c->walk_batches > 0)
+    (void)hipEventElapsedTime(&t_trav, c->ev_fork, c->ev_batch[1]);
+  c->early_ms[0] = t_pm > t_trav ? t_pm : t_trav;
+  c->early_ms[1] = t_pm;
+  c->early_ms[2] = t_trav;
+  c->last_pm_early = 1;
+  if(c->tune.pm_early < 0 && c->early_ms[0] > c->build_solo_ms + c->trav_solo_ms + c->pm_solo_ms)
+    c->pm_early_state = 0;
+  return NGRAVS_OK;
+}
+
 extern "C" int ngravs_compute_accelerations(ngravs_ctx *c, int pm_step)
 {
   if(!c || !c->have_particles)
@@ -1142,15 +1206,18 @@
   if((rc = domain_decomposition_impl(c, !(pm_step && c->cfg.pmgrid))))
     return rc;
   c->last_pm_cus = 0;
+  c->last_pm_early = 0;
   if(!(pm_step && c->cfg.pmgrid))
     return ngravs_gravity_tree(c);
+  if(choose_pm_early(c))
+    return early_step(c);
   const int R = choose_pm_cus(c);
   if(R > 0 && masked_streams(c, R) == NGRAVS_OK)
     {
       int64_t nn = ngravs_force_treebuild(c);
       if(nn < 0)
         return (int)nn;
-      if((rc = pm_on_masked_stream(c)))
+      if((rc = pm_on_stream(c, c->pm_stream, c->pm_stream_cus)))
         return rc;
       if((rc = gravity_tree_impl(c, c->ev_pm1)))
         return rc;
@@ -1170,6 +1237,8 @@
     {
       c->pm_solo_ms = c->stats.t_pm * 1e3;
       c->walk_solo_ms = c->stats.walk_kernel_ms;
+      c->build_solo_ms = c->stats.t_treebuild * 1e3;
+      c->trav_solo_ms = c->stats.reserved[6];
       c->pm_solo_steps++;
     }
   return NGRAVS_OK;
@@ -1416,6 +1485,80 @@
 extern "C" const char *ngravs_last_error(ngravs_ctx *c) { return c ? c->last_error.c_str() : g_create_error.c_str(); }
 extern "C" int ngravs_last_walk_kernel(ngravs_ctx *c) { return c ? c->last_walk_kernel : NGRAVS_ERR_ARG; }
 extern "C" int ngravs_last_pm_cus(ngravs_ctx *c) { return c ? c->last_pm_cus : NGRAVS_ERR_ARG; }
+
+extern "C" int ngravs_last_pm_early(ngravs_ctx *c, double phase_ms[3])
+{
+  if(!c)
+    return NGRAVS_ERR_ARG;
+  if(phase_ms)
+    for(int j = 0; j < 3; j++)
+      phase_ms[j] = c->last_pm_early ? c->early_ms[j] : 0.0;
+  return c->last_pm_early;
+}
+
+extern "C" int64_t ngravs_pm_patch_table(ngravs_ctx *c, int from_tree, int64_t cap, int32_t *first, int32_t *count, double *geo, int64_t *n_loose)
+{
+  if(!c || !c->have_order || !c->cfg.pmgrid || !c->cfg.periodic || c->n < 2)
+    return NGRAVS_ERR_STATE;
+  if(from_tree && (!c->have_tree || c->tree_stale))
+    return NGRAVS_ERR_STATE;
+  (void)hipSetDevice(c->cfg.device);
+  const int tl = pm_key_level(c, c->cfg.pmgrid / c->cfg.box_size);
+  if(tl < 0)
+    return 0;
+  std::vector<int> hf, hc;
+  std::vector<double> hg;
+  long long np = 0, loose = 0;
+  if(from_tree)
+    {
+      if(tl >= c->nlevels)
+        return 0;
+      const long long tl0 = c->level_start[tl];
+      np = c->level_start[tl + 1] - tl0;
+      hf.resize(np + 1), hc.resize(np + 1), hg.resize(4 * np + 4);
+      HIP_TRY(c, hipStreamSynchronize(c->stream));
+      HIP_TRY(c, hipMemcpy(hf.data(), c->n_first.p + tl0, sizeof(int) * np, hipMemcpyDeviceToHost));
+      HIP_TRY(c, hipMemcpy(hc.data(), c->n_count.p + tl0, sizeof(int) * np, hipMemcpyDeviceToHost));
+      HIP_TRY(c, hipMemcpy(hg.data(), c->n_geo.p + tl0, sizeof(double4) * np, hipMemcpyDeviceToHost));
+      std::vector<int> ch((size_t)8 * tl0 + 1);
+      HIP_TRY(c, hipMemcpy(ch.data(), c->n_child.p, sizeof(int) * 8 * tl0, hipMemcpyDeviceToHost));
+      for(long long t = 0; t < 8 * tl0; t++)
+        loose += ch[t] <= -2;
+    }
+  else
+    {
+      long long bound = 0;
+      int rc = pm_patches_from_keys(c, tl, &bound);
+      if(rc)
+        return rc;
+      HIP_TRY(c, hipStreamSynchronize(c->stream));
+      int hn = 0;
+      HIP_TRY(c, hipMemcpy(&hn, c->pmk_n.p, sizeof(int), hipMemcpyDeviceToHost));
+      if(hn < 0 || hn > bound)
+        return NGRAVS_ERR_TREE;
+      np = hn;
+      hf.resize(np + 1), hc.resize(np + 1), hg.resize(4 * np + 4);
+      HIP_TRY(c, hipMemcpy(hf.data(), c->pmk_first.p, sizeof(int) * np, hipMemcpyDeviceToHost));
+      HIP_TRY(c, hipMemcpy(hc.data(), c->pmk_count.p, sizeof(int) * np, hipMemcpyDeviceToHost));
+      HIP_TRY(c, hipMemcpy(hg.data(), c->pmk_geo.p, sizeof(double4) * np, hipMemcpyDeviceToHost));
+      const int ncell = 1 << (3 * tl);
+      std::vector<int> cc(ncell);
+      HIP_TRY(c, hipMemcpy(cc.data(), c->pmk_cell.p + ncell, sizeof(int) * ncell, hipMemcpyDeviceToHost));
+      for(int t = 0; t < ncell; t++)
+        loose += cc[t] == 1;
+    }
+  if(n_loose)
+    *n_loose = loose;
+  if(np > cap)
+    return NGRAVS_ERR_ARG;
+  if(first)
+    memcpy(first, hf.data(), sizeof(int) * np);
+  if(count)
+    memcpy(count, hc.data(), sizeof(int) * np);
+  if(geo)
+    memcpy(geo, hg.data(), sizeof(double) * 4 * np);
+  return np;
+}
 
 #define CU_PROBE_LDS (96 * 1024)
 __global__ void k_cu_probe(int *out, int n)
diff --git a/gadget-2.0.7-ngravs_amd/csrc/engine.hpp b/gadget-2.0.7-ngravs_amd/csrc/engine.hpp
--- a/gadget-2.0.7-ngravs_amd/csrc/engine.hpp
+++ b/gadget-2.0.7-ngravs_amd/csrc/engine.hpp
@@ -153,6 +153,7 @@
   int walk_ring = 1;
   int walk_ring_k = 0;
   int pm_cus = -1;
+  int pm_early = -1;
   int sph_verbose = 0;
 };
 
@@ -308,6 +309,16 @@
   int pm_solo_steps = 0;
   int pm_auto_cus = -1;
   hipEvent_t ev_fork = nullptr, ev_pm0 = nullptr, ev_pm1 = nullptr, ev_walk = nullptr;
+  hipStream_t early_stream = nullptr;
+  hipEvent_t eval_wait = nullptr;
+  int pm_early_state = -1;
+  int last_pm_early = 0;
+  double build_solo_ms = 0, trav_solo_ms = 0;
+  double early_ms[3] = {0, 0, 0};
+  DevBuf<int> pmk_cell;
+  DevBuf<int> pmk_first, pmk_count, pmk_n;
+  DevBuf<double4> pmk_geo;
+  DevBuf<unsigned char> pmk_tmp;
   DevBuf<int> probe_out;
   DevBuf<double> user_green;
   long long user_green_nk2 = 0;
@@ -445,6 +456,9 @@
 };
 int sph_hydro_run(ngravs_ctx *c, const SphHydroParams &hp, SphHydroStats *st);
 int sph_scatter(ngravs_ctx *c, const double *src, long long nt, double *dst, long long stride);
+static inline bool pm_keys_describe_tree(const ngravs_ctx *c) { return !c->top.on && !(c->have_tree && (c->tree_stale || c->tree_refit)); }
+int pm_key_level(const ngravs_ctx *c, double to_slab);
+int pm_patches_from_keys(ngravs_ctx *c, int tl, long long *bound);
 int pm_run(ngravs_ctx *c);
 int pm_deposit(ngravs_ctx *c);
 int pm_finish(ngravs_ctx *c);
diff --git a/gadget-2.0.7-ngravs_amd/csrc/kernels_pm.hip b/gadget-2.0.7-ngravs_amd/csrc/kernels_pm.hip
--- a/gadget-2.0.7-ngravs_amd/csrc/kernels_pm.hip
+++ b/gadget-2.0.7-ngravs_amd/csrc/kernels_pm.hip
@@ -1,6 +1,7 @@
 #include "engine.hpp"
 #include "pm_common.hpp"
 #include <hipfft/hipfft.h>
+#include <hipcub/hipcub.hpp>
 
 __global__ void k_cic_deposit(const double4 *__restrict__ s_pm, const unsigned char *__restrict__ s_type,
                               const unsigned char *__restrict__ s_flag, long long n,
@@ -226,10 +227,12 @@
 __global__ __launch_bounds__(PM_TILE_THREADS) void k_cic_deposit_tiled(
     const double4 *__restrict__ s_pm, const unsigned char *__restrict__ s_type, const unsigned char *__restrict__ s_flag,
     const int *__restrict__ n_first, const int *__restrict__ n_count, const double4 *__restrict__ n_geo, int node0,
-    double to_slab, int N, const int *__restrict__ t2g_tab, double *__restrict__ rho, MeshAddr ma)
+    const int *__restrict__ n_patches, double to_slab, int N, const int *__restrict__ t2g_tab, double *__restrict__ rho, MeshAddr ma)
 {
   constexpr int DT = PM_DT;
   extern __shared__ double tile[];
+  if(n_patches && (int)blockIdx.x >= *n_patches)
+    return;
   const int node = node0 + blockIdx.x;
   const double4 geo = n_geo[node];
   const int first = n_first[node], count = n_count[node];
@@ -317,6 +320,133 @@
   atomicAdd(&grid[ma.cell(sx + 1, sy + 1, sz + 1)], m * (dx)*dy * dz);
 }
 
+#define PM_KEY_LEVEL_MAX 8
+
+__device__ __forceinline__ int key_lower_bound(const unsigned long long *__restrict__ key, long long n, unsigned long long v)
+{
+  long long lo = 0, hi = n;
+  while(lo < hi)
+    {
+      const long long mid = (lo + hi) >> 1;
+      if(key[mid] < v)
+        lo = mid + 1;
+      else
+        hi = mid;
+    }
+  return (int)lo;
+}
+
+__global__ void k_pm_cells(const unsigned long long *__restrict__ key, long long n, int level, int ncell, int *__restrict__ cell_first,
+                           int *__restrict__ cell_count, int *__restrict__ is_node)
+{
+  const int cell = blockIdx.x * blockDim.x + threadIdx.x;
+  if(cell >= ncell)
+    return;
+  const int sh = 3 * (TREE_BITS - level);
+  const int a = key_lower_bound(key, n, (unsigned long long)cell << sh);
+  const int b = cell + 1 < ncell ? key_lower_bound(key, n, (unsigned long long)(cell + 1) << sh) : (int)n;
+  cell_first[cell] = a;
+  cell_count[cell] = b - a;
+  is_node[cell] = b - a >= 2 ? 1 : 0;
+}
+
+__global__ void k_pm_patches(const int *__restrict__ cell_first, const int *__restrict__ cell_count, const int *__restrict__ rank,
+                             int ncell, int level, const double4 *__restrict__ s_pm, double4 root, double cx, double cy, double cz,
+                             double fac21, int *__restrict__ tab_first, int *__restrict__ tab_count, double4 *__restrict__ tab_geo,
+                             int *__restrict__ n_patches)
+{
+  const int cell = blockIdx.x * blockDim.x + threadIdx.x;
+  if(cell >= ncell)
+    return;
+  const int cnt = cell_count[cell], r = rank[cell];
+  if(cell == ncell - 1)
+    *n_patches = r + (cnt >= 2 ? 1 : 0);
+  if(cnt < 2)
+    return;
+  const int first = cell_first[cell];
+  const double4 p = s_pm[first];
+  const int ix = (int)__dmul_rn(__dsub_rn(p.x, cx), fac21), iy = (int)__dmul_rn(__dsub_rn(p.y, cy), fac21),
+            iz = (int)__dmul_rn(__dsub_rn(p.z, cz), fac21);
+  double4 g = root;
+  for(int l = 1; l <= level; l++)
+    {
+      const int sh = TREE_BITS - l;
+      const double q = 0.25 * g.w;
+      g.x = ((ix >> sh) & 1) ? g.x + q : g.x - q;
+      g.y = ((iy >> sh) & 1) ? g.y + q : g.y - q;
+      g.z = ((iz >> sh) & 1) ? g.z + q : g.z - q;
+      g.w = 0.5 * g.w;
+    }
+  tab_first[r] = first;
+  tab_count[r] = cnt;
+  tab_geo[r] = g;
+}
+
+__global__ void k_cic_deposit_loose_cells(const double4 *__restrict__ s_pm, const unsigned char *__restrict__ s_type,
+                                          const unsigned char *__restrict__ s_flag, const int *__restrict__ cell_first,
+                                          const int *__restrict__ cell_count, int ncell, double to_slab, int N,
+                                          const int *__restrict__ t2g_tab, double *__restrict__ rho, MeshAddr ma)
+{
+  const int cell = blockIdx.x * blockDim.x + threadIdx.x;
+  if(cell >= ncell || cell_count[cell] != 1)
+    return;
+  const int i = cell_first[cell];
+  if(s_flag[i] & 2)
+    return;
+  double4 p = s_pm[i];
+  int g = t2g_tab[s_type[i]];
+  double *grid = rho + (size_t)g * ma.species_stride();
+  double dx, dy, dz;
+  int sx = cell_of(p.x, to_slab, N, &dx), sy = cell_of(p.y, to_slab, N, &dy), sz = cell_of(p.z, to_slab, N, &dz);
+  double m = p.w;
+  atomicAdd(&grid[ma.cell(sx, sy, sz)], m * (1.0 - dx) * (1.0 - dy) * (1.0 - dz));
+  atomicAdd(&grid[ma.cell(sx, sy + 1, sz)], m * (1.0 - dx) * dy * (1.0 - dz));
+  atomicAdd(&grid[ma.cell(sx, sy, sz + 1)], m * (1.0 - dx) * (1.0 - dy) * dz);
+  atomicAdd(&grid[ma.cell(sx, sy + 1, sz + 1)], m * (1.0 - dx) * dy * dz);
+  atomicAdd(&grid[ma.cell(sx + 1, sy, sz)], m * (dx) * (1.0 - dy) * (1.0 - dz));
+  atomicAdd(&grid[ma.cell(sx + 1, sy + 1, sz)], m * (dx)*dy * (1.0 - dz));
+  atomicAdd(&grid[ma.cell(sx + 1, sy, sz + 1)], m * (dx) * (1.0 - dy) * dz);
+  atomicAdd(&grid[ma.cell(sx + 1, sy + 1, sz + 1)], m * (dx)*dy * dz);
+}
+
+int pm_key_level(const ngravs_ctx *c, double to_slab)
+{
+  double len = c->dom[6];
+  for(int l = 0; l <= PM_KEY_LEVEL_MAX; l++, len *= 0.5)
+    if(len * to_slab <= 16.0 * 1.002)
+      return l;
+  return -1;
+}
+
+int pm_patches_from_keys(ngravs_ctx *c, int tl, long long *bound)
+{
+  const long long n = c->n;
+  const int ncell = 1 << (3 * tl);
+  const long long maxp = (long long)ncell < n / 2 ? (long long)ncell : n / 2;
+  size_t tmp_bytes = 0;
+  if(c->pmk_cell.ensure((size_t)4 * ncell) || c->pmk_first.ensure((size_t)maxp + 1) || c->pmk_count.ensure((size_t)maxp + 1) ||
+     c->pmk_geo.ensure((size_t)maxp + 1) || c->pmk_n.ensure(1))
+    return NGRAVS_ERR_NOMEM;
+  int *cell_first = c->pmk_cell.p, *cell_count = cell_first + ncell, *is_node = cell_count + ncell, *rank = is_node + ncell;
+  HIP_TRY(c, hipcub::DeviceScan::ExclusiveSum(nullptr, tmp_bytes, is_node, rank, ncell, c->stream));
+  if(c->pmk_tmp.ensure(tmp_bytes + 16))
+    return NGRAVS_ERR_NOMEM;
+  const unsigned nb = (unsigned)((ncell + 255) / 256);
+  hipLaunchKernelGGL(k_pm_cells, dim3(nb), dim3(256), 0, c->stream, c->s_key.p, n, tl, ncell, cell_first, cell_count, is_node);
+  HIP_TRY(c, hipcub::DeviceScan::ExclusiveSum(c->pmk_tmp.p, tmp_bytes, is_node, rank, ncell, c->stream));
+  double4 root;
+  root.x = c->dom[3];
+  root.y = c->dom[4];
+  root.z = c->dom[5];
+  root.w = c->dom[6];
+  const double fac21 = c->dom[7] * (double)(1 << (TREE_BITS - NGRAVS_BITS_PER_DIMENSION));
+  hipLaunchKernelGGL(k_pm_patches, dim3(nb), dim3(256), 0, c->stream, cell_first, cell_count, rank, ncell, tl, c->s_pm.p, root, c->dom[0],
+                     c->dom[1], c->dom[2], fac21, c->pmk_first.p, c->pmk_count.p, c->pmk_geo.p, c->pmk_n.p);
+  HIP_TRY(c, hipGetLastError());
+  *bound = maxp;
+  return NGRAVS_OK;
+}
+
 static int pm_tile_level(const ngravs_ctx *c, double to_slab)
 {
   if(!c->have_tree)
@@ -358,7 +488,7 @@
   auto launch_dep = [&](auto kern) -> int {
     HIP_TRY(c, hipFuncSetAttribute(reinterpret_cast<const void *>(kern), hipFuncAttributeMaxDynamicSharedMemorySize, (int)lds));
     hipLaunchKernelGGL(kern, dim3((unsigned)tln), dim3(PM_TILE_THREADS), lds, c->stream, c->s_pm.p, c->s_type.p, c->s_active.p,
-                       c->n_first.p, c->n_count.p, c->n_geo.p, (int)tl0, to_slab, N, c->d_counters.p + 8, dst, ma);
+                       c->n_first.p, c->n_count.p, c->n_geo.p, (int)tl0, (const int *)nullptr, to_slab, N, c->d_counters.p + 8, dst, ma);
     return NGRAVS_OK;
   };
   const int rc = ng == 1 ? launch_dep(k_cic_deposit_tiled<1>) : (ng == 2 ? launch_dep(k_cic_deposit_tiled<2>) : launch_dep(k_cic_deposit_tiled<3>));
@@ -367,6 +497,39 @@
   if(tl0 > 0)
     hipLaunchKernelGGL(k_cic_deposit_loose, dim3((unsigned)((8 * tl0 + bs - 1) / bs)), dim3(bs), 0, c->stream, c->s_pm.p, c->s_type.p,
                        c->s_active.p, c->n_child.p, (int)tl0, to_slab, N, c->d_counters.p + 8, dst, ma);
+  HIP_TRY(c, hipGetLastError());
+  return NGRAVS_OK;
+}
+
+static int pm_deposit_tiles_keys(ngravs_ctx *c, const MeshAddr &ma, double *dst)
+{
+  const int N = c->cfg.pmgrid, ng = c->cfg.n_gravs;
+  const double to_slab = N / c->cfg.box_size;
+  const int bs = 256;
+  const int tl = c->n >= 2 ? pm_key_level(c, to_slab) : -1;
+  if(tl < 0)
+    return 1;
+  long long bound = 0;
+  int rc = pm_patches_from_keys(c, tl, &bound);
+  if(rc)
+    return rc;
+  const int ncell = 1 << (3 * tl);
+  const size_t lds = sizeof(double) * ng * PM_DT * PM_DT * PM_DT;
+  auto launch_dep = [&](auto kern) -> int {
+    HIP_TRY(c, hipFuncSetAttribute(reinterpret_cast<const void *>(kern), hipFuncAttributeMaxDynamicSharedMemorySize, (int)lds));
+    hipLaunchKernelGGL(kern, dim3((unsigned)bound), dim3(PM_TILE_THREADS), lds, c->stream, c->s_pm.p, c->s_type.p, c->s_active.p,
+                       c->pmk_first.p, c->pmk_count.p, c->pmk_geo.p, 0, (const int *)c->pmk_n.p, to_slab, N, c->d_counters.p + 8, dst, ma);
+    return NGRAVS_OK;
+  };
+  if(bound > 0)
+    {
+      rc = ng == 1 ? launch_dep(k_cic_deposit_tiled<1>) : (ng == 2 ? launch_dep(k_cic_deposit_tiled<2>) : launch_dep(k_cic_deposit_tiled<3>));
+      if(rc)
+        return rc;
+    }
+  if(tl > 0)
+    hipLaunchKernelGGL(k_cic_deposit_loose_cells, dim3((unsigned)((ncell + bs - 1) / bs)), dim3(bs), 0, c->stream, c->s_pm.p, c->s_type.p,
+                       c->s_active.p, c->pmk_cell.p, c->pmk_cell.p + ncell, ncell, to_slab, N, c->d_counters.p + 8, dst, ma);
   HIP_TRY(c, hipGetLastError());
   return NGRAVS_OK;
 }
@@ -407,7 +570,7 @@
       ma.lo[j] = 0;
       ma.ext[j] = N;
     }
-  int rct = pm_deposit_tiles(c, ma, c->pm_rho.p);
+  int rct = pm_keys_describe_tree(c) ? pm_deposit_tiles_keys(c, ma, c->pm_rho.p) : pm_deposit_tiles(c, ma, c->pm_rho.p);
   if(rct == 1)
     hipLaunchKernelGGL(k_cic_deposit, dim3(nbp), dim3(bs), 0, c->stream, c->s_pm.p, c->s_type.p, c->s_active.p, n, to_slab, N, ng,
                        c->d_counters.p + 8, c->pm_rho.p);
diff --git a/gadget-2.0.7-ngravs_amd/csrc/kernels_walk.hip b/gadget-2.0.7-ngravs_amd/csrc/kernels_walk.hip
--- a/gadget-2.0.7-ngravs_amd/csrc/kernels_walk.hip
+++ b/gadget-2.0.7-ngravs_amd/csrc/kernels_walk.hip
@@ -2358,6 +2358,8 @@
                          walk_tcount(c), c->walk_counters.p, (int *)nullptr, c->walk_counters.p + 1, c->r_acc.p,
                          c->r_nint.p, region, gcount, u0, nbu, lcap, scap, c->walk_ovf.p, S, G, walk_tlist(c), SG);
       HIP_TRY(c, hipEventRecord(c->ev_batch[3 * ib + 1], c->stream));
+      if(c->eval_wait)
+        HIP_TRY(c, hipStreamWaitEvent(c->stream, c->eval_wait, 0));
       if(g0 > 0)
         HIP_TRY(c, hipMemsetAsync(c->walk_counters.p + 8, 0, sizeof(int) * 8, c->stream));
       long long nblk = ncu;
diff --git a/include/ngravs_hip.h b/include/ngravs_hip.h
--- a/include/ngravs_hip.h
+++ b/include/ngravs_hip.h
@@ -148,6 +148,8 @@
                                int nlat, ngravs_ctx **out);
 int ngravs_last_walk_kernel(ngravs_ctx *ctx);
 int ngravs_last_pm_cus(ngravs_ctx *ctx);
+int ngravs_last_pm_early(ngravs_ctx *ctx, double phase_ms[3]);
+int64_t ngravs_pm_patch_table(ngravs_ctx *ctx, int from_tree, int64_t cap, int32_t *first, int32_t *count, double *geo, int64_t *n_loose);
 int ngravs_cu_probe(ngravs_ctx *ctx, int which, int nblocks, int32_t *cu_ids);
 void ngravs_destroy(ngravs_ctx *ctx);
 void ngravs_set_fatal_handler(ngravs_ctx *ctx, ngravs_fatal_fn fn);
```

Measured after the change: 608.8 million. 2.4% lower.
